# 5l1v3r1/gr-dvbt2ll

Hardware: NVIDIA B200
Metric: t2_baseband_msps (higher is better)
Workload: dtype u8/f32

## Files before the change

gr-dvbt2ll_b200/csrc/t2_capi.cu:

```cuda
#include "../../include/dvbt2ll_cuda.h"

#include <cuda_runtime.h>

#include <algorithm>
#include <cmath>
#include <cstdio>
#include <cstdlib>
#include <cstring>
#include <memory>
#include <mutex>
#include <string>
#include <vector>

#include "t2_kernels.cuh"
#include "t2_plan.h"

namespace {

thread_local std::string g_err;

int fail(int code, const std::string &msg) { g_err = msg; return code; }

#define CK(call)                                                                                  \
  do {                                                                                            \
// ... 280 lines not shown
struct BbHandle : dvbt2ll_handle {
  t2::BbPlan plan;
  DevBuf d_scr, d_crc, d_tab, d_cols, d_ib, d_ts, d_packed;
  int count, fec_block;
  uint8_t history[187];
  long long total_consumed;
  int *h_err;
  BbHandle() : dvbt2ll_handle(BB), count(0), fec_block(0), total_consumed(0), h_err(0) { std::memset(history, 0, sizeof(history)); }
  ~BbHandle() { if (h_err) cudaFreeHost(h_err); }
  void note_consumed(const uint8_t *in, long long used)
  {
    if (used >= 187) std::memcpy(history, in + used - 187, 187);
    else if (used > 0) {
      std::memmove(history, history + used, 187 - (size_t)used);
      std::memcpy(history + 187 - used, in, (size_t)used);
    }
  }

  int output_multiple() const { return plan.fec.nbch; }
  int in_item() const { return 1; }
  int out_item() const { return 1; }
  int forecast(int noutput) const
  {
    const int base = (noutput - 80 - (plan.fec.nbch - plan.fec.kbch)) / 8;
    return plan.mode == t2::INPUTMODE_NORMAL ? base : base + ((plan.fec.kbch - 80) / 8) / 187 + 1;
  }
  uint32_t crc_pos_mask[47][8];
  int dev_init()
  {
    std::vector<uint8_t> scr(plan.scramble);
    scr.resize((scr.size() + 7) & ~(size_t)3, 0);
    CK(upload(d_scr, scr));
    CK(upload(d_crc, std::vector<uint8_t>(plan.crc8_tab, plan.crc8_tab + 256)));
    std::vector<uint8_t> crc(1024);
    for (int x = 0; x < 256; x++) {
      uint8_t v = plan.crc8_tab[x];
      for (int k = 0; k < 4; k++) { crc[k * 256 + x] = v; v = plan.crc8_tab[v]; }
    }
    uint32_t crc_mask[8];
    for (int k = 0; k < 8; k++) {
      crc_mask[k] = 0;
      for (int i = 0; i < 4; i++)
        for (int j = 0; j < 8; j++)
          if ((crc[(3 - i) * 256 + (1 << j)] >> k) & 1) crc_mask[k] |= 1u << (8 * i + j);
    }
    {
      auto step = [&](uint32_t t) { uint32_t c = 0; for (int k = 0; k < 8; k++) c |= (uint32_t)(__builtin_popcount(t & crc_mask[k]) & 1) << k; return c; };
      std::memset(crc_pos_mask, 0, sizeof(crc_pos_mask));
      for (int j = 0; j < 47; j++)
        for (int bit = 0; bit < 32; bit++) {
          uint32_t v = step(1u << bit);
          for (int r = 0; r < 46 - j; r++) v = step(v);
          for (int k = 0; k < 8; k++) if ((v >> k) & 1u) crc_pos_mask[j][k] |= 1u << bit;
        }
      for (int k = 0; k < 8; k++) crc_pos_mask[0][k] &= 0xFFFFFF00u;
    }
    CK(upload(d_tab, plan.bch_byte_tab));
    CK(upload(d_cols, plan.bch_shift_cols));
    CK(upload(d_ib, plan.inband_bytes));
    if (!h_err) {
      CK(cudaHostAlloc((void **)&h_err, 16, cudaHostAllocMapped | cudaHostAllocPortable));
      std::memset(h_err, 0, 16);
    }
    return 0;
  }
  long long payload_bytes(int frames, int fb0) const
  {
    long long nb = 0;
    if (plan.inband) nb = (fb0 + frames + plan.fecblocks - 1) / plan.fecblocks - (fb0 + plan.fecblocks - 1) / plan.fecblocks;
    return (long long)frames * plan.payload_bytes - 13 * nb;
  }
  long long ts_needed(int frames) const
  {
    const long long P = payload_bytes(frames, fec_block);
    if (plan.mode == t2::INPUTMODE_NORMAL || P == 0) return P;
    const int t0 = (188 - count) % 188;
    const long long last = P - 1;
    return (last < t0 ? last : t0 + 1 + (last - t0) + (last - t0) / 187) + 1;
  }
  void fill_args(t2k::BbArgs &a, const uint8_t *d_ts_ptr, long long pitch, int channels, int frames, int count0,
                 int fb0, int hist_valid, uint8_t *d_out, int out_pitch)
  {
    a.ts = d_ts_ptr; a.ts_pitch = pitch; a.hist_valid = hist_valid; a.n_channels = channels; a.frames = frames;
    a.count0 = count0; a.fec_block0 = fb0;
    a.kbch = plan.fec.kbch; a.nbch = plan.fec.nbch; a.bch_r = plan.fec.bch_r; a.payload_bytes = plan.payload_bytes;
    a.mode = plan.mode; a.inband = plan.inband ? 1 : 0; a.fecblocks = plan.fecblocks;
    a.chunk_bytes = plan.chunk_bytes; a.lead_zero_bytes = plan.lead_zero_bytes;
    a.scramble = d_scr.as<uint8_t>(); a.crc8_tab = d_crc.as<uint8_t>(); a.bch_tab = d_tab.as<uint32_t>();
    std::memcpy(a.crc8_pos_mask, crc_pos_mask, sizeof(crc_pos_mask));
    a.bch_cols = d_cols.as<uint32_t>(); a.inband_bytes = d_ib.as<uint8_t>();
    a.out = d_out; a.out_pitch = out_pitch; a.sync_errors = h_err;
    a.ts_len = 0; a.out_len = (long long)channels * frames * out_pitch;
    a.out_group = 0; a.out_group_stride = 0; a.out_group_off = 0;
  }
  int work_device(const void *d_in, int ninput, void *d_out, int noutput, int *consumed, cudaStream_t s)
  {
    const int frames = noutput / plan.fec.nbch;
    if (consumed) *consumed = 0;
    if (frames < 1) return 0;
    const long long need = ts_needed(frames);
    if (ninput < need) return fail(DVBT2LL_ERR_SHORT, "bbheaderbch_bb: not enough input items");
    const int pitch = align16(plan.fec.nbch / 8);
    CK(d_packed.ensure((size_t)frames * pitch));
    t2k::BbArgs a;
    fill_args(a, (const uint8_t *)d_in, 0, 1, frames, count, fec_block, hist_on_device, d_packed.as<uint8_t>(), pitch);
    a.ts_len = ninput;
    t2k::launch_bb_bch(a, s);
    t2k::launch_unpack_bits(d_packed.as<uint8_t>(), pitch, plan.fec.nbch, (uint8_t *)d_out, frames, s);
    CK(cudaGetLastError());
    count = (int)((count + need) % 188);
    if (plan.inband) fec_block = (fec_block + frames) % plan.fecblocks;
    total_consumed += need;
    if (consumed) *consumed = (int)need;
    return frames * plan.fec.nbch;
  }
  int hist_on_device = 0;
  long long plan_get(const char *name, void *out, long long cap) const
  {
    std::string n(name);
    if (n == "bb.scramble") return copy_vec(plan.scramble, out, cap);
    if (n == "bb.crc8") return copy_out(plan.crc8_tab, 256, out, cap);
    if (n == "bb.bch_tab") return copy_vec(plan.bch_byte_tab, out, cap);
    if (n == "bb.bch_cols") return copy_vec(plan.bch_shift_cols, out, cap);
    if (n == "bb.inband") return copy_vec(plan.inband_bytes, out, cap);
    if (n == "bb.dims") {
      const int v[8] = { plan.fec.kbch, plan.fec.nbch, plan.fec.q, plan.fec.bch_r, plan.payload_bytes,
                         plan.chunk_bytes, plan.lead_zero_bytes, plan.fec.nldpc };
      return copy_out(v, sizeof(v), out, cap);
    }
    return -1;
  }
};

struct LdpcHandle : dvbt2ll_handle {
  t2::LdpcPlan plan;
  DevBuf d_rowptr, d_entries, d_in_packed, d_out_packed;
  int lane_per_row;
  LdpcHandle() : dvbt2ll_handle(LDPC), lane_per_row(0) {}
  int output_multiple() const { return plan.fec.nldpc; }
  int in_item() const { return 1; }
  int out_item() const { return 1; }
  int forecast(int noutput) const { return (noutput / plan.fec.nldpc) * plan.fec.nbch; }
  int dev_init()
  {
    CK(upload(d_rowptr, plan.row_ptr));
    CK(upload(d_entries, plan.entries));
    lane_per_row = ldpc_lane_per_row_default(plan.fec.nldpc, plan.fec.q);
    const char *e = std::getenv("DVBT2LL_LDPC_MODE");
    if (e && (e[0] == '0' || e[0] == '1')) lane_per_row = e[0] - '0';
    return 0;
  }
  static int ldpc_lane_per_row_default(int nldpc, int q)
  {
    return nldpc == 64800 ? (q >= 90 ? 1 : 0) : (q >= 18 ? 1 : 0);
  }
  void fill_args(t2k::LdpcArgs &a, const uint8_t *in, int in_pitch, uint8_t *out, int out_pitch, int frames)
  {
    a.in = in; a.in_pitch = in_pitch; a.out = out; a.out_pitch = out_pitch; a.frames = frames;
    a.nbch = plan.fec.nbch; a.nldpc = plan.fec.nldpc; a.q = plan.fec.q; a.groups = plan.groups;
    a.row_ptr = d_rowptr.as<uint16_t>(); a.entries = d_entries.as<uint32_t>();
    a.lane_per_row = lane_per_row;
    a.in_len = (long long)frames * in_pitch + 64; a.out_len = (long long)frames * out_pitch;
  }
  int work_device(const void *d_in, int ninput, void *d_out, int noutput, int *consumed, cudaStream_t s)
  {
    const int frames = noutput / plan.fec.nldpc;
    if (consumed) *consumed = 0;
    if (frames < 1) return 0;
    if (ninput < frames * plan.fec.nbch) return fail(DVBT2LL_ERR_SHORT, "ldpc: not enough input items");
    const int ip = align16(plan.fec.nbch / 8), op = align16(plan.fec.nldpc / 8);
    CK(d_in_packed.ensure((size_t)frames * ip + 64));
    CK(d_out_packed.ensure((size_t)frames * op + 16));
    t2k::launch_pack_bits((const uint8_t *)d_in, plan.fec.nbch, d_in_packed.as<uint8_t>(), ip, frames, s);
    t2k::LdpcArgs a;
    fill_args(a, d_in_packed.as<uint8_t>(), ip, d_out_packed.as<uint8_t>(), op, frames);
    t2k::launch_ldpc(a, s);
    t2k::launch_unpack_ldpc(d_out_packed.as<uint8_t>(), op, plan.fec.nbch, plan.fec.nldpc, plan.fec.q, (uint8_t *)d_out, frames, s);
    CK(cudaGetLastError());
    if (consumed) *consumed = frames * plan.fec.nbch;
    return frames * plan.fec.nldpc;
  }
  long long plan_get(const char *name, void *out, long long cap) const
  {
    std::string n(name);
    if (n == "ldpc.row_ptr") return copy_vec(plan.row_ptr, out, cap);
    if (n == "ldpc.entries") return copy_vec(plan.entries, out, cap);
    return -1;
  }
};

struct MapHandle : dvbt2ll_handle {
  t2::MapPlan plan;
  DevBuf d_bitsrc, d_lut, d_packed, d_qlut;
  MapHandle() : dvbt2ll_handle(MAP) {}
  int output_multiple() const { return plan.cell_size; }
  int in_item() const { return 1; }
  int out_item() const { return 8; }
  int forecast(int noutput) const { return (noutput / plan.cell_size) * plan.fec.nldpc; }
  int dev_init()
  {
    CK(upload(d_bitsrc, plan.bit_src));
    CK(upload(d_lut, plan.lut));
    if (!plan.qpsk_lut.empty()) CK(upload(d_qlut, plan.qpsk_lut));
    return 0;
  }
  void fill_args(t2k::MapArgs &a, const uint8_t *in, int in_pitch, float2 *out, int frames)
  {
    a.in = in; a.in_pitch = in_pitch; a.out = out; a.frames = frames;
    a.nldpc = plan.fec.nldpc; a.mod = plan.mod; a.cell_size = plan.cell_size; a.cyclic_delay = plan.cyclic_delay;
    a.bit_src = d_bitsrc.as<uint16_t>(); a.lut = d_lut.as<float2>();
    a.qpsk_lut = plan.qpsk_lut.empty() ? 0 : d_qlut.as<uint2>(); a.qpsk_lin_cells = a.qpsk_lut ? plan.qpsk_lin_cells : 0;
    a.qpsk_par_q = a.qpsk_lut ? plan.qpsk_par_q : 0; a.qpsk_nbch = plan.qpsk_nbch;
    a.ci_inv = 0; a.ci_inv4 = 0; a.ci_inv4_stride = 0; a.fec_shift = 0; a.fecblocks = 1; a.out16 = 0; a.out16_frame_stride = 0;
    a.in_len = (long long)frames * in_pitch; a.out_len = 0;
    a.ncol = plan.ncol;
    a.im_from_re = plan.im_from_re; a.im_mask_i = plan.im_mask_i; a.im_mask_q = plan.im_mask_q; a.im_flip = plan.im_flip;
    std::memcpy(a.col_of_bit, plan.col_of_bit, 16);
    std::memcpy(a.twist_of_col, plan.twist_of_col, 16);
  }
  int work_device(const void *d_in, int ninput, void *d_out, int noutput, int *consumed, cudaStream_t s)
  {
    const int frames = noutput / plan.cell_size;
    if (consumed) *consumed = 0;
    if (frames < 1) return 0;
    if (ninput < frames * plan.fec.nldpc) return fail(DVBT2LL_ERR_SHORT, "interleavermod_bc: not enough input items");
    const int ip = align16(plan.fec.nldpc / 8);
    CK(d_packed.ensure((size_t)frames * ip + 16));
    t2k::launch_pack_ldpc((const uint8_t *)d_in, plan.fec.nbch, plan.fec.nldpc, plan.fec.q, d_packed.as<uint8_t>(), ip, frames, s);
    t2k::MapArgs a;
    fill_args(a, d_packed.as<uint8_t>(), ip, (float2 *)d_out, frames);
    t2k::launch_map(a, s);
    CK(cudaGetLastError());
    if (consumed) *consumed = frames * plan.fec.nldpc;
    return frames * plan.cell_size;
  }
  long long plan_get(const char *name, void *out, long long cap) const
  {
    std::string n(name);
    if (n == "map.bit_src") return copy_vec(plan.bit_src, out, cap);
    if (n == "map.lut") return copy_vec(plan.lut, out, cap);
    if (n == "map.qpsk") { const int v[3] = { plan.qpsk_lin_cells, plan.qpsk_par_q, plan.qpsk_nbch }; return copy_out(v, sizeof(v), out, cap); }
    if (n == "map.im_from_re") { const int v[4] = { plan.im_from_re, (int)plan.im_mask_i, (int)plan.im_mask_q, (int)plan.im_flip }; return copy_out(v, sizeof(v), out, cap); }
    return -1;
  }
};

struct FrameHandle : dvbt2ll_handle {
  t2::FramePlan plan;
  DevBuf d_code, d_pool;
  int t2_frame_num;
  FrameHandle() : dvbt2ll_handle(FRAME), t2_frame_num(0) {}
  int output_multiple() const { return plan.mapped_items; }
  int in_item() const { return 8; }
  int out_item() const { return 8; }
  int forecast(int noutput) const { return plan.stream_items * (noutput / plan.mapped_items); }
  int dev_init()
  {
    CK(upload(d_code, plan.code));
    CK(upload(d_pool, plan.pool.cells));
    return 0;
  }
  int work_device(const void *d_in, int ninput, void *d_out, int noutput, int *consumed, cudaStream_t s)
  {
    const int frames = noutput / plan.mapped_items;
    if (consumed) *consumed = 0;
    if (frames < 1) return 0;
    if ((long long)ninput < (long long)frames * plan.stream_items)
      return fail(DVBT2LL_ERR_SHORT, "framemapperfint_cc: not enough input items");
    t2k::GatherArgs a;
    a.in = (const float2 *)d_in; a.in_stride = plan.stream_items;
    a.out = (float2 *)d_out; a.out_stride = plan.mapped_items;
    a.code = d_code.as<int32_t>(); a.n = plan.mapped_items; a.pool = d_pool.as<float2>();
    a.l1post_base = plan.pool.l1post_base; a.l1post_cells = plan.pool.l1post_cells; a.l1post_variants = plan.pool.l1post_variants;
    a.frames = frames; a.frame_idx0 = t2_frame_num;
    t2k::launch_gather(a, s);
    CK(cudaGetLastError());
    t2_frame_num = (t2_frame_num + frames) % plan.prm.t2frames;
    if (consumed) *consumed = frames * plan.stream_items;
    return frames * plan.mapped_items;
  }
  long long plan_get(const char *name, void *out, long long cap) const
  {
    std::string n(name);
    if (n == "frame.code") return copy_vec(plan.code, out, cap);
    if (n == "frame.pool") return copy_vec(plan.pool.cells, out, cap);
    if (n == "frame.cell_perm") return copy_vec(plan.cell_perm, out, cap);
    if (n == "frame.fec_shift") return copy_vec(plan.fec_shift, out, cap);
    if (n == "frame.ci_dst") return copy_vec(plan.ci_dst, out, cap);
    if (n == "frame.ti_src") return copy_vec(plan.ti_src, out, cap);
    if (n == "frame.dims") return dims_get(plan.dims, out, cap);
    if (n == "frame.info") {
      const int v[12] = { plan.cell_size, plan.stream_items, plan.mapped_items, plan.eta_mod, plan.n_post, plan.n_punc,
                          plan.dummy_cells, plan.pool.l1post_base, plan.pool.l1post_cells, plan.pool.l1post_variants,
                          plan.pool_dummy, plan.pool_zero };
      return copy_out(v, sizeof(v), out, cap);
    }
    return -1;
  }
};

struct OfdmDevice {
  DevBuf d_code, d_pool, d_p1, d_sinc, d_tw, d_tw_split, d_sym_flags;
  int log2_m, split;
  long long pool_stride;
  int init(const std::vector<int32_t> &code, const t2::CellPool &pool, const t2::OfdmPlan &op, bool c16 = false,
           const std::vector<uint8_t> *plp = 0, const int *tab_base = 0)
  {
    {
      const int nv = pool.l1post_variants > 0 ? pool.l1post_variants : 1;
      pool_stride = (long long)pool.cells.size();
      std::vector<t2::cfloat> rep((size_t)nv * pool.cells.size());
      for (int v = 0; v < nv; v++) {
        std::copy(pool.cells.begin(), pool.cells.end(), rep.begin() + (size_t)v * pool.cells.size());
        for (int i = 0; i < pool.l1post_cells; i++)
          rep[(size_t)v * pool.cells.size() + pool.l1post_base + i] = pool.cells[pool.l1post_base + (size_t)v * pool.l1post_cells + i];
      }
      CK(upload(d_pool, rep));
    }
    CK(upload(d_p1, op.p1));
    const int N = op.dims.fft_n;
    split = N > 16384 ? 2 : 1;
    const int M = N / split;
    log2_m = 0;
    while ((1 << log2_m) < M) log2_m++;
    const int L = op.dims.num_symbols, cps = op.dims.c_ps;
    std::vector<int> pos(M);
    for (int m = 0; m < M; m++) pos[m] = t2k::ofdm_table_index(t2k::ofdm_position_of_bin(m, log2_m), log2_m);
    std::vector<int32_t> code_pos((size_t)L * N, -1);
    std::vector<int32_t> sym_flags(L, 0);
// ... 96 lines not shown
  std::vector<uint16_t> c4((size_t)4 * *stride, 0);
  for (int k = 0; k < 4; k++)
    for (int j = 0; j + k < nc; j++) {
      const int c = ci_inv[j + k];
      c4[(size_t)k * *stride + j] = (uint16_t)(c + 2 * (c >> 6));
    }
  return c4;
}

struct ChainHandle : dvbt2ll_handle {
  BbHandle bb;
  LdpcHandle ldpc;
  MapHandle map;
  struct Set { BbHandle bb; LdpcHandle ldpc; MapHandle map; };
  std::unique_ptr<Set> xset[t2::MAX_PLP];
  DevBuf d_ci_inv_p[t2::MAX_PLP], d_ci_inv4_p[t2::MAX_PLP];
  int ci4_stride_p[t2::MAX_PLP];
  size_t bch_off[t2::MAX_PLP + 1], fec_off[t2::MAX_PLP + 1];
  std::vector<t2::cfloat> luts;
  int lut_tables, lut_base[t2::MAX_PLP], lut_single;
  int lut_copies;
  DevBuf d_luts;
  t2::FramePlan fplan;
  t2::OfdmPlan oplan;
  t2::Chain16Tables tables;
  OfdmDevice odev;
  DevBuf d_bch, d_fec, d_cells, d_ts_stage, d_out_stage, d_ci_inv, d_ci_inv4, d_fec_shift, d_run_desc, d_run_ptr, d_run_cnt, d_stage_bytes;
  int stage_cap, ci4_stride;
  int max_frames, device;
  int sink_fmt;
  float sink_gain;
  cudaStream_t stream2;
  int tr_iter;
  float tr_vclip, tr_tone_max;
  bool tr_built, tr_uploaded;
  t2::PaprTrPlan tr;
  DevBuf d_tr_set, d_tr_bins, d_tr_kernel, d_tr_tw, d_tr_stats, d_tr_scratch;
  int tr_frames;
  int last_frames;
  long long next_frame;
  bool timing;
  enum { TIMING_SLOTS = 64 };
  cudaEvent_t ev[TIMING_SLOTS][5];
  long long n_timed;
  ChainHandle() : dvbt2ll_handle(CHAIN), lut_tables(1), lut_single(0), lut_copies(0), max_frames(0), device(0), sink_fmt(0), sink_gain(1.0f), stream2(0), tr_iter(0), tr_vclip(0.f), tr_tone_max(0.f), tr_built(false), tr_uploaded(false), tr_frames(0), last_frames(0), next_frame(0), timing(false)
  {
    n_timed = 0;
    for (int s = 0; s < TIMING_SLOTS; s++) for (int i = 0; i < 5; i++) ev[s][i] = 0;
  }
  ~ChainHandle()
  {
    for (int s = 0; s < TIMING_SLOTS; s++) for (int i = 0; i < 5; i++) if (ev[s][i]) cudaEventDestroy(ev[s][i]);
    if (stream2) cudaStreamDestroy(stream2);
  }
  int enter() override
  {
    if (device >= 0) CK(cudaSetDevice(device));
    return ensure_device();
  }
  bool mixed() const { return fplan.plp_sets > 1; }
  BbHandle &bb_of(int plp) { const int s = fplan.plp_set[plp]; return s ? xset[s]->bb : bb; }
  const BbHandle &bb_of(int plp) const { const int s = fplan.plp_set[plp]; return s ? xset[s]->bb : bb; }
  LdpcHandle &ldpc_of(int plp) { const int s = fplan.plp_set[plp]; return s ? xset[s]->ldpc : ldpc; }
  MapHandle &map_of(int plp) { const int s = fplan.plp_set[plp]; return s ? xset[s]->map : map; }
  int bch_pitch(int plp) const { return align16(bb_of(plp).plan.fec.nbch / 8); }
  int fec_pitch(int plp) const { return align16(bb_of(plp).plan.fec.nldpc / 8); }
  int F() const { return fplan.prm.fecblocks; }
  int P() const { return fplan.num_plp; }
  int Fp(int plp) const { return fplan.plp_first_block[plp + 1] - fplan.plp_first_block[plp]; }
  long long cells16_stride() const { return ((long long)fplan.plp_chain_off[P()] + 7) & ~7LL; }
  long long stream_pos(long long frame, int plp = 0) const
  {
    const int fpl = Fp(plp);
    const long long j0 = frame * fpl;
    long long nb0 = 0;
    if (bb.plan.inband) nb0 = (j0 + fpl - 1) / fpl;
    const long long P = j0 * bb_of(plp).plan.payload_bytes - 13 * nb0;
    if (bb.plan.mode == t2::INPUTMODE_NORMAL || P == 0) return P;
    const long long last = P - 1;
    return 1 + last + last / 187 + 1;
  }
  long long ts_bytes(long long first_frame, int n_frames, int plp = 0) const { return stream_pos(first_frame + n_frames, plp) - stream_pos(first_frame, plp); }
  long long ts_bytes_max(long long first_frame, int n_frames) const
  {
    long long m = 0;
    for (int pl = 0; pl < P(); pl++) m = std::max(m, ts_bytes(first_frame, n_frames, pl));
    return m;
  }
  long long ts_per_frame() const { return ts_bytes(0, 1); }
  int output_multiple() const { return oplan.samples_per_frame; }
  int in_item() const { return 1; }
  int out_item() const { return sink_fmt ? 4 : 8; }
  int forecast(int noutput) const { return (int)(ts_per_frame() * (noutput / oplan.samples_per_frame)); }
  int dev_init()
  {
    bb.stream = 0; ldpc.stream = 0; map.stream = 0;
    int r;
    if ((r = bb.dev_init())) return r;
    if ((r = ldpc.dev_init())) return r;
    if ((r = map.dev_init())) return r;
    for (int s = 1; s < fplan.plp_sets; s++) {
      Set &x = *xset[s];
      x.bb.stream = 0; x.ldpc.stream = 0; x.map.stream = 0;
      if ((r = x.bb.dev_init()) || (r = x.ldpc.dev_init()) || (r = x.map.dev_init())) return r;
    }
    if ((r = odev.init(tables.code, tables.pool, oplan, true, &tables.plp, lut_tables > 1 ? lut_base : 0))) return r;
    CK(upload(d_ci_inv, fplan.cell_perm_inv));
    CK(upload(d_ci_inv4, make_ci_inv4(fplan.cell_perm_inv, &ci4_stride)));
    if (mixed()) {
      for (int pl = 0; pl < P(); pl++) {
        CK(upload(d_ci_inv_p[pl], fplan.plp_cell_perm_inv[pl]));
        CK(upload(d_ci_inv4_p[pl], make_ci_inv4(fplan.plp_cell_perm_inv[pl], &ci4_stride_p[pl])));
      }
      CK(upload(d_luts, luts));
    }
    CK(upload(d_fec_shift, fplan.fec_shift));
    CK(upload(d_run_desc, tables.run_desc));
    CK(upload(d_run_ptr, tables.run_ptr));
    CK(upload(d_run_cnt, tables.run_cnt));
    CK(upload(d_stage_bytes, tables.stage_bytes));
    stage_cap = (tables.max_slots + 7) & ~7;
    if ((size_t)(1 << odev.log2_m) * 8 * 17 / 16 + (size_t)stage_cap * 2 + 2048 + 96 + (size_t)(tables.max_runs + 2) * 8 > 227 * 1024)
      return fail(DVBT2LL_ERR_INVALID, "chain: the cells of one OFDM symbol do not fit the shared-memory staging area");
    const size_t nfec = (size_t)max_frames * F();
    bch_off[0] = fec_off[0] = 0;
    for (int pl = 0; pl < P(); pl++) {
      bch_off[pl + 1] = bch_off[pl] + (size_t)max_frames * Fp(pl) * bch_pitch(pl);
      fec_off[pl + 1] = fec_off[pl] + (size_t)max_frames * Fp(pl) * fec_pitch(pl);
    }
    if (mixed()) {
      CK(d_bch.ensure(bch_off[P()] + 64));
      CK(d_fec.ensure(fec_off[P()] + 64));
    }
    else CK(d_bch.ensure(nfec * align16(bb.plan.fec.nbch / 8) + 64));
    CK(d_cells.ensure((size_t)max_frames * cells16_stride() * sizeof(uint16_t) + 64));
    CK(cudaMemset(d_cells.p, 0, (size_t)max_frames * cells16_stride() * sizeof(uint16_t) + 64));
    for (int s = 0; s < TIMING_SLOTS; s++) for (int i = 0; i < 5; i++) CK(cudaEventCreate(&ev[s][i]));
    return 0;
  }
  int run(const void *d_ts, long long ts_pitch, int n_channels, int n_frames, long long first_frame, void *d_out, cudaStream_t s,
          int buf_frame = 0, int hist_valid = -1, int tr_frame0 = 0)
  {
    const int frames = n_channels * n_frames;
    if (frames < 1) return 0;
    if (buf_frame + frames > max_frames) return fail(DVBT2LL_ERR_INVALID, "chain: batch larger than max_frames given at create");
    const int nfec = frames * F();
    const int bp = align16(bb.plan.fec.nbch / 8), fp = align16(bb.plan.fec.nldpc / 8);
    cudaEvent_t *tev = ev[n_timed % TIMING_SLOTS];
    if (timing) cudaEventRecord(tev[0], s);
    uint8_t *bch_buf = d_bch.as<uint8_t>() + (size_t)buf_frame * F() * bp;
    if (!mixed()) CK(d_fec.ensure((size_t)max_frames * F() * fp + 64));
    uint8_t *fec_buf = d_fec.as<uint8_t>() + (size_t)buf_frame * F() * fp;
    uint16_t *cell_buf = d_cells.as<uint16_t>() + (size_t)buf_frame * cells16_stride();
    if (mixed()) run_plps(d_ts, ts_pitch, n_channels, n_frames, first_frame, cell_buf, s, buf_frame, hist_valid, tev);
    else {
    for (int pl = 0; pl < P(); pl++) {
      const int fpl = Fp(pl);
      const long long j0 = first_frame * fpl;
      const int fb0 = bb.plan.inband ? (int)(j0 % fpl) : 0;
      const int count0 = (int)(stream_pos(first_frame, pl) % 188);
      t2k::BbArgs ba;
      bb.fill_args(ba, (const uint8_t *)d_ts + (long long)pl * ts_pitch, ts_pitch * P(), n_channels, n_frames * fpl, count0, fb0,
                   hist_valid >= 0 ? hist_valid : (first_frame > 0 ? 1 : 0), bch_buf, bp);
      ba.fecblocks = fpl;
      ba.ts_len = ts_bytes(first_frame, n_frames, pl);
      ba.out_len = (long long)frames * F() * bp;
      if (P() > 1) { ba.out_group = fpl; ba.out_group_stride = F(); ba.out_group_off = fplan.plp_first_block[pl]; }
      t2k::launch_bb_bch(ba, s);
    }
    if (timing) cudaEventRecord(tev[1], s);
    t2k::LdpcArgs la;
    ldpc.fill_args(la, bch_buf, bp, fec_buf, fp, nfec);
    t2k::MapArgs ma;
    map.fill_args(ma, fec_buf, fp, 0, nfec);
    ma.out16 = cell_buf; ma.out16_frame_stride = cells16_stride();
    ma.ci_inv = d_ci_inv.as<uint16_t>(); ma.fec_shift = d_fec_shift.as<int32_t>(); ma.fecblocks = F();
    ma.ci_inv4 = d_ci_inv4.as<uint16_t>(); ma.ci_inv4_stride = ci4_stride;
    ma.out_len = (long long)frames * cells16_stride();
    t2k::launch_ldpc(la, s);
    if (timing) cudaEventRecord(tev[2], s);
    t2k::launch_map(ma, s);
    if (timing) cudaEventRecord(tev[3], s);
    }
    const bool tr_on = tr_iter > 0, tr_inplace = tr_on && sink_fmt == 0 && sink_gain == 1.0f;
    const long long spf = oplan.samples_per_frame;
    void *ofdm_out = d_out;
    if (tr_on) {
      int r = tr_upload();
      if (r) return r;
      CK(d_tr_stats.ensure((size_t)(tr_frame0 + frames) * oplan.dims.num_symbols * sizeof(int16_t)));
      if (!tr_inplace) {
        CK(d_tr_scratch.ensure((size_t)max_frames * spf * sizeof(float2)));
        ofdm_out = d_tr_scratch.as<float2>() + (size_t)buf_frame * spf;
      }
    }
    t2k::OfdmArgs oa;
    odev.fill(oa, oplan, tables.pool);
    oa.cells = 0; oa.cells_stride = cells16_stride();
    oa.cells16 = cell_buf; oa.run_desc = d_run_desc.as<int2>(); oa.run_ptr = d_run_ptr.as<int32_t>();
    oa.run_cnt = d_run_cnt.as<int32_t>(); oa.desc_cap = (tables.max_runs + 2) & ~1;
    oa.stage_bytes = d_stage_bytes.as<int32_t>(); oa.stage_cap = stage_cap; oa.lut_single = map.plan.im_from_re;
    oa.lut = map.d_lut.as<float2>(); oa.lut_n = 1 << map.plan.mod;
    if (mixed()) { oa.lut_single = lut_single; oa.lut = d_luts.as<float2>(); oa.lut_n = (int)luts.size(); oa.lut_tables = lut_tables; }
    oa.out = ofdm_out; oa.out_stride = oplan.samples_per_frame;
    oa.cells_len = (long long)frames * cells16_stride(); oa.out_len = (long long)frames * oplan.samples_per_frame;
    oa.out_fmt = sink_fmt; oa.sink_gain = sink_gain; oa.norm = oplan.normalization * sink_gain;
    if (ofdm_out != d_out) { oa.out_fmt = 0; oa.sink_gain = 1.0f; oa.norm = oplan.normalization; }
    oa.frames = frames; oa.frames_per_channel = n_frames;
    oa.frame_idx0 = (int)(first_frame % (tables.pool.l1post_variants > 0 ? tables.pool.l1post_variants : 1));
    lut_copies = t2k::launch_ofdm(oa, s);
    if (tr_on) {
      t2k::PaprArgs pa;
      pa.in = (const float2 *)ofdm_out; pa.out = d_out;
      pa.out_fmt = sink_fmt; pa.gain = sink_gain; pa.inplace = tr_inplace ? 1 : 0;
      pa.spf = spf; pa.fft_n = oplan.dims.fft_n; pa.gi = oplan.dims.gi; pa.num_symbols = oplan.dims.num_symbols; pa.frames = frames;
      pa.iterations = tr_iter; pa.vclip = tr_vclip; pa.tone_max = tr_tone_max;
      pa.tone_scale = (float)(1.0 / ((double)oplan.normalization * tr.tones));
      pa.tones = tr.tones; pa.sets = tr.sets;
      pa.sym_set = d_tr_set.as<int32_t>(); pa.bins = d_tr_bins.as<int32_t>();
      pa.kernel = d_tr_kernel.as<float2>(); pa.tone_tw = d_tr_tw.as<float2>();
      pa.stats = d_tr_stats.as<int16_t>() + (size_t)tr_frame0 * oplan.dims.num_symbols;
      pa.in_len = pa.out_len = (long long)frames * spf;
      t2k::launch_papr_tr(pa, s);
      tr_frames = tr_frame0 + frames;
    }
    if (timing) { cudaEventRecord(tev[4], s); n_timed++; }
    CK(cudaGetLastError());
    if (buf_frame == 0) last_frames = frames;
    return frames;
  }
  int tr_upload()
  {
    if (tr_uploaded) return 0;
    CK(upload(d_tr_set, tr.sym_set));
    CK(upload(d_tr_bins, tr.bins));
    CK(upload(d_tr_kernel, tr.kernel));
    CK(upload(d_tr_tw, tr.tone_tw));
    tr_uploaded = true;
    return 0;
  }
  void run_plps(const void *d_ts, long long ts_pitch, int n_channels, int n_frames, long long first_frame, uint16_t *cell_buf,
                cudaStream_t s, int buf_frame, int hist_valid, cudaEvent_t *tev)
  {
    const int frames = n_channels * n_frames;
    auto bch_buf = [&](int pl) { return d_bch.as<uint8_t>() + bch_off[pl] + (size_t)buf_frame * Fp(pl) * bch_pitch(pl); };
    auto fec_buf = [&](int pl) { return d_fec.as<uint8_t>() + fec_off[pl] + (size_t)buf_frame * Fp(pl) * fec_pitch(pl); };
    for (int pl = 0; pl < P(); pl++) {
      const int fpl = Fp(pl);
      const long long j0 = first_frame * fpl;
      t2k::BbArgs ba;
      bb_of(pl).fill_args(ba, (const uint8_t *)d_ts + (long long)pl * ts_pitch, ts_pitch * P(), n_channels, n_frames * fpl,
                          (int)(stream_pos(first_frame, pl) % 188), bb.plan.inband ? (int)(j0 % fpl) : 0,
                          hist_valid >= 0 ? hist_valid : (first_frame > 0 ? 1 : 0), bch_buf(pl), bch_pitch(pl));
      ba.fecblocks = fpl;
      ba.ts_len = ts_bytes(first_frame, n_frames, pl);
      t2k::launch_bb_bch(ba, s);
    }
    if (timing) cudaEventRecord(tev[1], s);
    for (int pl = 0; pl < P(); pl++) {
      t2k::LdpcArgs la;
      ldpc_of(pl).fill_args(la, bch_buf(pl), bch_pitch(pl), fec_buf(pl), fec_pitch(pl), frames * Fp(pl));
      t2k::launch_ldpc(la, s);
    }
    if (timing) cudaEventRecord(tev[2], s);
    for (int pl = 0; pl < P(); pl++) {
      t2k::MapArgs ma;
      map_of(pl).fill_args(ma, fec_buf(pl), fec_pitch(pl), 0, frames * Fp(pl));
      ma.out16 = cell_buf + fplan.plp_chain_off[pl]; ma.out16_frame_stride = cells16_stride();
      ma.ci_inv = d_ci_inv_p[pl].as<uint16_t>(); ma.fec_shift = d_fec_shift.as<int32_t>() + fplan.plp_first_block[pl];
      ma.fecblocks = Fp(pl);
      ma.ci_inv4 = d_ci_inv4_p[pl].as<uint16_t>(); ma.ci_inv4_stride = ci4_stride_p[pl];
      ma.im_from_re = lut_single;
      ma.out_len = (long long)frames * cells16_stride() - fplan.plp_chain_off[pl];
      t2k::launch_map(ma, s);
    }
    if (timing) cudaEventRecord(tev[3], s);
  }
  int work_device(const void *d_in, int ninput, void *d_out, int noutput, int *consumed, cudaStream_t s)
  {
    const int frames = noutput / oplan.samples_per_frame;
    if (consumed) *consumed = 0;
    if (frames < 1) return 0;
    const long long need = ts_bytes(next_frame, frames);
    if ((long long)ninput < need) return fail(DVBT2LL_ERR_SHORT, "chain: not enough input items");
    int r = run(d_in, 0, 1, frames, next_frame, d_out, s);
    if (r < 0) return r;
    next_frame += frames;
    if (consumed) *consumed = (int)need;
    return frames * oplan.samples_per_frame;
  }
  long long plan_get(const char *name, void *out, long long cap) const
  {
    std::string n(name);
    if (n == "chain.code") return copy_vec(tables.code, out, cap);
    if (n == "chain.pool") return copy_vec(tables.pool.cells, out, cap);
    if (n == "chain.run_desc") return copy_vec(tables.run_desc, out, cap);
    if (n == "chain.run_ptr") return copy_vec(tables.run_ptr, out, cap);
    if (n == "chain.run_cnt") return copy_vec(tables.run_cnt, out, cap);
    if (n == "chain.stage_bytes") return copy_vec(tables.stage_bytes, out, cap);
    if (n == "ofdm.sym_data_start") return copy_vec(oplan.sym_data_start, out, cap);
    if (n == "frame.framed") return copy_vec(fplan.framed, out, cap);
    if (n == "frame.pool") return copy_vec(fplan.pool.cells, out, cap);
    if (n == "frame.info") {
      const int v[12] = { fplan.cell_size, fplan.stream_items, fplan.mapped_items, fplan.eta_mod, fplan.n_post, fplan.n_punc,
                          fplan.dummy_cells, fplan.pool.l1post_base, fplan.pool.l1post_cells, fplan.pool.l1post_variants,
                          fplan.pool_dummy, fplan.pool_zero };
      return copy_out(v, sizeof(v), out, cap);
    }
    if (n == "frame.plp") {
      int v[2 + t2::MAX_PLP + 1] = { fplan.num_plp, fplan.l1post_sig_bits };
      for (int i = 0; i <= fplan.num_plp; i++) v[2 + i] = fplan.plp_first_block[i];
      return copy_out(v, sizeof(int) * (3 + fplan.num_plp), out, cap);
    }
    if (n == "frame.fi_src") return copy_vec(fplan.fi_src, out, cap);
    if (tr_built && n == "ofdm.tr_set") return copy_vec(tr.sym_set, out, cap);
    if (tr_built && n == "ofdm.tr_bins") return copy_vec(tr.bins, out, cap);
    if (tr_built && n == "ofdm.tr_kernel") return copy_vec(tr.kernel, out, cap);
    if (n == "frame.fec_shift") return copy_vec(fplan.fec_shift, out, cap);
    if (n == "frame.plp_cells") {
      int v[3 * t2::MAX_PLP];
      for (int i = 0; i < P(); i++) { v[3 * i] = fplan.plp_cell_size[i]; v[3 * i + 1] = fplan.plp_first_cell[i]; v[3 * i + 2] = fplan.plp_chain_off[i]; }
      return copy_out(v, sizeof(int) * 3 * P(), out, cap);
    }
    if (n == "chain.luts") {
      int v[3 + t2::MAX_PLP] = { lut_tables, mixed() ? lut_single : map.plan.im_from_re, lut_copies };
      for (int i = 0; i < P(); i++) v[3 + i] = mixed() ? lut_base[i] : 0;
      return copy_out(v, sizeof(int) * (3 + P()), out, cap);
    }
    long long r;
    if ((r = bb.plan_get(name, out, cap)) >= 0) return r;
    if ((r = ldpc.plan_get(name, out, cap)) >= 0) return r;
    if ((r = map.plan_get(name, out, cap)) >= 0) return r;
    if (n == "frame.code") return copy_vec(fplan.code, out, cap);
    if (n == "frame.ci_dst") return copy_vec(fplan.ci_dst, out, cap);
    if (n == "ofdm.code") return copy_vec(oplan.code, out, cap);
    if (n == "ofdm.dims") return dims_get(oplan.dims, out, cap);
    return -1;
  }
};

}

extern "C" {

const char *dvbt2ll_last_error(void) { return g_err.c_str(); }
#ifdef DVBT2LL_DEBUG_BOUNDS
const char *dvbt2ll_version(void) { return "dvbt2ll-b200 0.2 (sm_100a, bounds-checking debug build)"; }
#else
const char *dvbt2ll_version(void) { return "dvbt2ll-b200 0.2 (sm_100a)"; }
#endif
long long dvbt2ll_kernel_launches(void) { return t2k::kernel_launch_count(); }

int dvbt2ll_device_available(void)
{
  int n = 0;
  if (cudaGetDeviceCount(&n) != cudaSuccess) { cudaGetLastError(); return 0; }
  return n > 0;
}

int dvbt2ll_output_multiple(const dvbt2ll_handle *h) { return h ? h->output_multiple() : DVBT2LL_ERR_INVALID; }
int dvbt2ll_forecast(const dvbt2ll_handle *h, int noutput) { return h ? h->forecast(noutput) : DVBT2LL_ERR_INVALID; }
int dvbt2ll_warnings(const dvbt2ll_handle *h) { return h ? h->warnings : 0; }
void dvbt2ll_destroy(dvbt2ll_handle *h) { delete h; }

long long dvbt2ll_plan_get(const dvbt2ll_handle *h, const char *name, void *out, long long cap)
{
  if (!h || !name) return -1;
  return h->plan_get(name, out, cap);
}

int dvbt2ll_work_device(dvbt2ll_handle *h, const void *d_in, int ninput, void *d_out, int noutput, int *consumed, void *stream)
{
  if (!h) return fail(DVBT2LL_ERR_INVALID, "null handle");
  int r = h->enter();
  if (r) return r;
  if (h->kind == dvbt2ll_handle::BB) {
    BbHandle *b = static_cast<BbHandle *>(h);
    b->hist_on_device = b->total_consumed > 0 ? 1 : 0;
  }
  cudaStream_t s = stream ? (cudaStream_t)stream : h->stream;
  r = h->work_device(d_in, ninput, d_out, noutput, consumed, s);
  if (r >= 0 && !stream) CK(cudaStreamSynchronize(s));
  return r;
}

int dvbt2ll_work(dvbt2ll_handle *h, const void *in, int ninput, void *out, int noutput, int *consumed)
{
  if (!h) return fail(DVBT2LL_ERR_INVALID, "null handle");
  if (consumed) *consumed = 0;
  int r = h->enter();
  if (r) return r;
  const int om = h->output_multiple();
  const int frames = noutput / om;
  if (frames < 1) return 0;
  const int nout = frames * om;
  BbHandle *b = h->kind == dvbt2ll_handle::BB ? static_cast<BbHandle *>(h) : 0;
  ChainHandle *ch = h->kind == dvbt2ll_handle::CHAIN ? static_cast<ChainHandle *>(h) : 0;
  if (ch && ch->P() > 1) return fail(DVBT2LL_ERR_INVALID, "chain: a multi-PLP chain takes one TS per PLP: use dvbt2ll_chain_run_host / _run_device");
  if (ch) b = &ch->bb;
  long long need;
  if (ch) need = ch->ts_bytes(ch->next_frame, frames);
  else if (b) need = b->ts_needed(frames);
  else need = (long long)h->forecast(nout);
  if (ninput < need) return fail(DVBT2LL_ERR_SHORT, "not enough input items for the requested output");
  if (ch && frames > ch->max_frames) return fail(DVBT2LL_ERR_INVALID, "chain: more frames requested than max_frames given at create");
  DevBuf &d_in = h->stage_in;
  const size_t in_bytes = (size_t)need * h->in_item(), out_bytes = (size_t)nout * h->out_item();
  const size_t prefix = 192;
  std::shared_ptr<LinkRec> found_in = h->link_in;
  std::unique_lock<std::mutex> lk_in, lk_out;
  const bool auto_link = !ch && AutoLinks::get().enabled();
  if (auto_link && !h->link_out) {
    h->link_out = std::make_shared<LinkRec>();
    h->link_out->item = h->out_item();
    AutoLinks::get().add(h->link_out);
  }
  if (!found_in && auto_link && !b) {
    const uint8_t *ip = (const uint8_t *)in;
    std::vector<std::shared_ptr<LinkRec> > cand;
    if (std::shared_ptr<LinkRec> last = h->auto_in.lock()) cand.push_back(last);
    const size_t tried_first = cand.size();
    for (int pass = 0; pass < 2 && !found_in; pass++) {
      if (pass == 1) AutoLinks::get().snapshot(cand);
      for (size_t i = pass ? tried_first : 0; i < cand.size() && !found_in; i++) {
        LinkRec &L = *cand[i];
        if (cand[i] == h->link_out || L.item != h->in_item()) continue;
        std::unique_lock<std::mutex> g(L.m);
        for (int k = 0; k < LinkRec::NSLOT; k++) {
          const LinkRec::Slot &S = L.slot[k];
// ... 71 lines not shown
    b->hist_on_device = 1;
  }
  if (!resident) CK(h->copy_host(din, in, in_bytes, cudaMemcpyHostToDevice, s));
  int used = 0;
  if (ch) {
    r = ch->run(din, 0, 1, frames, ch->next_frame, d_out.p, s, 0, 1);
    if (r >= 0) { r = nout; used = (int)need; ch->next_frame += frames; }
  }
  else r = h->work_device(din, (int)need, d_out.p, nout, &used, s);
  if (r < 0) return r;
  if (resident) {
    if (!taken->taken_ev) CK(cudaEventCreateWithFlags(&taken->taken_ev, cudaEventDisableTiming));
    CK(cudaEventRecord(taken->taken_ev, s));
    taken->taken_valid = true;
    lk_in.unlock();
  }
  const bool lazy_out = h->link_out && h->link_out->lazy;
  if (!lazy_out) CK(h->copy_host(out, d_out.p, out_bytes, cudaMemcpyDeviceToHost, s));
  CK(cudaStreamSynchronize(s));
  if (b) {
    h->warnings = *b->h_err;
    b->note_consumed((const uint8_t *)in, used);
  }
  if (mine) {
    lk_out.lock();
    LinkRec &L = *h->link_out;
    mine->host = (const uint8_t *)out; mine->bytes = out_bytes; mine->valid = true;
    mine->pending = lazy_out; mine->taken_to = 0;
    L.next = (L.next + 1) % LinkRec::NSLOT;
  }
  if (consumed) *consumed = used;
  return r;
}

long long dvbt2ll_ts_sync(const unsigned char *ts, size_t n)
{
  if (!ts) return -1;
  for (size_t off = 0; off < 188 && off < n; off++) {
    int ok = 0;
    size_t q = off;
    for (; q < n && ok < 5; q += 188, ok++)
      if (ts[q] != 0x47) break;
    if (ok == 5 || (ok > 0 && q >= n)) return (long long)off;
  }
  return -1;
}
long long dvbt2ll_ts_fill(unsigned char *dst, size_t dst_bytes, const unsigned char *src, size_t src_bytes, long long pos)
{
  if (!dst) return -1;
  const long long whole = (long long)(src_bytes / 188) * 188;
  long long nulls = 0;
  for (size_t i = 0; i < dst_bytes; i++) {
    const long long q = pos + (long long)i;
    if (q < 0) dst[i] = 0;
    else if (q < whole && src) dst[i] = src[q];
    else {
      const int k = (int)(q % 188);
      dst[i] = k == 0 ? 0x47 : k == 1 ? 0x1F : k == 2 ? 0xFF : k == 3 ? 0x10 : 0xFF;
      nulls++;
    }
  }
  return nulls;
}

int dvbt2ll_copy_to_host(void *dst, const void *d_src, size_t bytes)
{
  CK(cudaMemcpy(dst, d_src, bytes, cudaMemcpyDeviceToHost));
  return 0;
}
int dvbt2ll_copy_to_device(void *d_dst, const void *src, size_t bytes)
{
  CK(cudaMemcpy(d_dst, src, bytes, cudaMemcpyHostToDevice));
  return 0;
}
void *dvbt2ll_device_alloc(size_t bytes)
{
  void *p = 0;
  if (cudaMalloc(&p, bytes) != cudaSuccess) { fail(DVBT2LL_ERR_CUDA, std::string("cudaMalloc: ") + cudaGetErrorString(cudaGetLastError())); return 0; }
  return p;
}
void dvbt2ll_device_free(void *p) { if (p) cudaFree(p); }
int dvbt2ll_device_count(void)
{
  int n = 0;
  if (cudaGetDeviceCount(&n) != cudaSuccess) { cudaGetLastError(); return 0; }
  return n;
}
int dvbt2ll_set_device(int device) { CK(cudaSetDevice(device)); return 0; }
void *dvbt2ll_stream_create(void)
{
  cudaStream_t s = 0;
  if (cudaStreamCreateWithFlags(&s, cudaStreamNonBlocking) != cudaSuccess) { fail(DVBT2LL_ERR_CUDA, "cudaStreamCreate failed"); cudaGetLastError(); return 0; }
  return (void *)s;
}
void dvbt2ll_stream_destroy(void *stream) { if (stream) cudaStreamDestroy((cudaStream_t)stream); }
int dvbt2ll_stream_synchronize(void *stream) { CK(cudaStreamSynchronize((cudaStream_t)stream)); return 0; }
int dvbt2ll_device_synchronize(void) { CK(cudaDeviceSynchronize()); return 0; }

void dvbt2ll_set_overfull_policy(int policy) { t2::set_overfull_policy(policy); }

void dvbt2ll_set_host_register(dvbt2ll_handle *h, int on) { if (h) h->pin_enabled = on != 0; }

int dvbt2ll_link(dvbt2ll_handle *producer, dvbt2ll_handle *consumer)
{
  if (!producer || !consumer || producer == consumer) return fail(DVBT2LL_ERR_INVALID, "link: two distinct handles needed");
  if (producer->out_item() != consumer->in_item()) return fail(DVBT2LL_ERR_INVALID, "link: item sizes differ");
  if (consumer->kind == dvbt2ll_handle::BB || consumer->kind == dvbt2ll_handle::CHAIN)
    return fail(DVBT2LL_ERR_INVALID, "link: a TS-consuming block keeps stream history in front of its input and cannot be a consumer");
  std::shared_ptr<LinkRec> L = std::make_shared<LinkRec>();
  L->item = producer->out_item();
  producer->link_out = L;
  consumer->link_in = L;
  return 0;
}

long long dvbt2ll_link_hits(const dvbt2ll_handle *consumer)
{
  if (!consumer) return 0;
  return consumer->link_in ? consumer->link_in->hits : consumer->auto_hits;
}

void dvbt2ll_set_auto_link(int on)
{
  AutoLinks &a = AutoLinks::get();
  std::lock_guard<std::mutex> g(a.m);
  a.on = on ? 1 : 0;
}

int dvbt2ll_link_lazy_host(dvbt2ll_handle *producer, int on)
{
  if (!producer || !producer->link_out) return fail(DVBT2LL_ERR_INVALID, "link_lazy_host: the handle is not the producer of a link");
  std::lock_guard<std::mutex> g(producer->link_out->m);
  producer->link_out->lazy = on != 0;
  return 0;
}

long long dvbt2ll_link_late_writes(const dvbt2ll_handle *producer) { return (producer && producer->link_out) ? producer->link_out->late_writes : 0; }

dvbt2ll_handle *dvbt2ll_bbheaderbch_create(int framesize, int rate, int mode, int inband, int fecblocks, int tsrate)
{
  BbHandle *h = new BbHandle();
  std::string err;
  if (mode != t2::INPUTMODE_NORMAL && mode != t2::INPUTMODE_HIEFF) { delete h; fail(DVBT2LL_ERR_INVALID, "bbheaderbch_bb: unknown input mode"); return 0; }
  if (!t2::build_bb_plan(framesize, rate, mode, inband, fecblocks, tsrate, &h->plan, &err)) { delete h; fail(DVBT2LL_ERR_INVALID, err); return 0; }
  return h;
}

dvbt2ll_handle *dvbt2ll_ldpc_create(int framesize, int rate)
{
  LdpcHandle *h = new LdpcHandle();
  std::string err;
  if (!t2::build_ldpc_plan(framesize, rate, &h->plan, &err)) { delete h; fail(DVBT2LL_ERR_INVALID, err); return 0; }
  return h;
}

dvbt2ll_handle *dvbt2ll_interleavermod_create(int framesize, int rate, int constellation, int rotation)
{
  MapHandle *h = new MapHandle();
  std::string err;
  if (!t2::build_map_plan(framesize, rate, constellation, rotation, &h->plan, &err)) { delete h; fail(DVBT2LL_ERR_INVALID, err); return 0; }
  return h;
}

dvbt2ll_handle *dvbt2ll_framemapperfint_create(int framesize, int rate, int constellation, int rotation, int fecblocks,
                                               int tiblocks, int carriermode, int fftsize, int guardinterval,
                                               int l1constellation, int pilotpattern, int t2frames, int numdatasyms,
                                               int paprmode, int version, int preamble, int inputmode,
                                               int reservedbiasbits, int l1scrambled, int inband)
{
  FrameHandle *h = new FrameHandle();
  std::string err;
  t2::FrameParams p = { framesize, rate, constellation, rotation, fecblocks, tiblocks, carriermode, fftsize, guardinterval,
                        l1constellation, pilotpattern, t2frames, numdatasyms, paprmode, version, preamble, inputmode,
                        reservedbiasbits, l1scrambled, inband };
  if (!t2::build_frame_plan(p, &h->plan, &err)) { delete h; fail(DVBT2LL_ERR_INVALID, err); return 0; }
  if (h->plan.overfull) { h->warnings = 1; g_err = "Frame Mapper, too many FEC blocks in T2 frame."; }
  return h;
}

dvbt2ll_handle *dvbt2ll_pilotgenp1insert_create(int carriermode, int fftsize, int pilotpattern, int guardinterval,
                                                int numdatasyms, int paprmode, int version, int preamble,
                                                int misogroup, int equalization, int bandwidth, int vlength)
{
  OfdmHandle *h = new OfdmHandle();
  std::string err;
  t2::OfdmParams p = { carriermode, fftsize, pilotpattern, guardinterval, numdatasyms, paprmode, version, preamble,
                       misogroup, equalization, bandwidth, vlength };
  if (!t2::build_ofdm_plan(p, &h->plan, &err)) { delete h; fail(DVBT2LL_ERR_INVALID, err); return 0; }
  return h;
}

static dvbt2ll_handle *chain_create(const dvbt2ll_chain_params *c, int num_plp, const int *plp_fecblocks, int max_frames, int device)
{
  if (!c || max_frames < 1) { fail(DVBT2LL_ERR_INVALID, "chain: bad arguments"); return 0; }
  if (num_plp < 1 || num_plp > t2::MAX_PLP || (num_plp > 1 && !plp_fecblocks)) { fail(DVBT2LL_ERR_INVALID, "chain: number of PLPs out of range"); return 0; }
  ChainHandle *h = new ChainHandle();
  std::string err;
  h->max_frames = max_frames; h->device = device;
  int fecblocks = c->fecblocks;
  if (num_plp > 1) {
    fecblocks = 0;
    for (int p = 0; p < num_plp; p++) fecblocks += plp_fecblocks[p];
  }
  t2::FrameParams fp = { c->framesize, c->rate, c->constellation, c->rotation, fecblocks, c->tiblocks, c->carriermode,
                         c->fftsize, c->guardinterval, c->l1constellation, c->pilotpattern, c->t2frames, c->numdatasyms,
                         c->paprmode, c->version, c->preamble, c->inputmode, c->reservedbiasbits, c->l1scrambled, c->inband };
  fp.num_plp = num_plp;
  for (int p = 0; p < num_plp && num_plp > 1; p++) fp.plp_fecblocks[p] = plp_fecblocks[p];
  t2::OfdmParams op = { c->carriermode, c->fftsize, c->pilotpattern, c->guardinterval, c->numdatasyms, c->paprmode,
                        c->version, c->preamble, c->misogroup, c->equalization, c->bandwidth, c->vlength };
  bool ok = true;
  ok = ok && t2::build_bb_plan(c->framesize, c->rate, c->inputmode, c->inband, fecblocks, c->tsrate, &h->bb.plan, &err);
  ok = ok && t2::build_ldpc_plan(c->framesize, c->rate, &h->ldpc.plan, &err);
  ok = ok && t2::build_map_plan(c->framesize, c->rate, c->constellation, c->rotation, &h->map.plan, &err);
  ok = ok && t2::build_frame_plan(fp, &h->fplan, &err);
  ok = ok && t2::build_ofdm_plan(op, &h->oplan, &err);
  ok = ok && t2::compose_chain16(h->fplan, h->oplan, &h->tables, &err);
  if (!ok) { delete h; fail(DVBT2LL_ERR_INVALID, err); return 0; }
  if (h->fplan.overfull) { h->warnings = 1; g_err = "Frame Mapper, too many FEC blocks in T2 frame."; }
  return h;
}

dvbt2ll_handle *dvbt2ll_chain_create_plps(const dvbt2ll_chain_params *c, int num_plp, const dvbt2ll_plp_params *plp, int max_frames,
                                          int device)
{
  if (!c || !plp || max_frames < 1) { fail(DVBT2LL_ERR_INVALID, "chain: bad arguments"); return 0; }
  if (num_plp < 1 || num_plp > t2::MAX_PLP) { fail(DVBT2LL_ERR_INVALID, "chain: number of PLPs out of range"); return 0; }
  int fecblocks = 0;
  for (int p = 0; p < num_plp; p++) {
    if (plp[p].fecblocks < 1 || plp[p].fecblocks > 1023) { fail(DVBT2LL_ERR_INVALID, "chain: FEC blocks of a PLP out of range"); return 0; }
    fecblocks += plp[p].fecblocks;
  }
  std::unique_ptr<ChainHandle> h(new ChainHandle());
  std::string err;
  h->max_frames = max_frames; h->device = device;
  t2::FrameParams fp = { plp[0].framesize, plp[0].rate, plp[0].constellation, plp[0].rotation, fecblocks, c->tiblocks,
                         c->carriermode, c->fftsize, c->guardinterval, c->l1constellation, c->pilotpattern, c->t2frames,
                         c->numdatasyms, c->paprmode, c->version, c->preamble, c->inputmode, c->reservedbiasbits,
                         c->l1scrambled, c->inband };
  fp.num_plp = num_plp;
  fp.plp_modcod = 1;
  for (int p = 0; p < num_plp; p++) {
    fp.plp_fecblocks[p] = plp[p].fecblocks;
    fp.plp_framesize[p] = plp[p].framesize; fp.plp_rate[p] = plp[p].rate;
    fp.plp_constellation[p] = plp[p].constellation; fp.plp_rotation[p] = plp[p].rotation;
  }
  t2::OfdmParams op = { c->carriermode, c->fftsize, c->pilotpattern, c->guardinterval, c->numdatasyms, c->paprmode,
                        c->version, c->preamble, c->misogroup, c->equalization, c->bandwidth, c->vlength };
  bool ok = t2::build_frame_plan(fp, &h->fplan, &err);
  for (int s = 0; ok && s < h->fplan.plp_sets; s++) {
    int p = 0;
    while (h->fplan.plp_set[p] != s) p++;
    if (s) h->xset[s].reset(new ChainHandle::Set());
    BbHandle &bb = s ? h->xset[s]->bb : h->bb;
    LdpcHandle &ldpc = s ? h->xset[s]->ldpc : h->ldpc;
    MapHandle &map = s ? h->xset[s]->map : h->map;
    ok = ok && t2::build_bb_plan(plp[p].framesize, plp[p].rate, c->inputmode, c->inband, fecblocks, c->tsrate, &bb.plan, &err);
    ok = ok && t2::build_ldpc_plan(plp[p].framesize, plp[p].rate, &ldpc.plan, &err);
    ok = ok && t2::build_map_plan(plp[p].framesize, plp[p].rate, plp[p].constellation, plp[p].rotation, &map.plan, &err);
  }
  ok = ok && t2::build_ofdm_plan(op, &h->oplan, &err);
  ok = ok && t2::compose_chain16(h->fplan, h->oplan, &h->tables, &err);
  if (!ok) { fail(DVBT2LL_ERR_INVALID, err); return 0; }
  if (h->mixed()) {
    std::vector<int> order;
    for (int p = 0; p < num_plp; p++) order.push_back(p);
    std::stable_sort(order.begin(), order.end(), [&](int x, int y) { return plp[x].constellation > plp[y].constellation; });
    h->lut_tables = 0;
    h->lut_single = 1;
    for (size_t i = 0; i < order.size(); i++) {
      const int p = order[i];
      const t2::MapPlan &mp = h->map_of(p).plan;
      h->lut_single &= mp.im_from_re;
      size_t j = 0;
      while (j < i && !(plp[order[j]].constellation == plp[p].constellation && plp[order[j]].rotation == plp[p].rotation)) j++;
      if (j < i) { h->lut_base[p] = h->lut_base[order[j]]; continue; }
      h->lut_base[p] = (int)h->luts.size();
      h->luts.insert(h->luts.end(), mp.lut.begin(), mp.lut.end());
      h->lut_tables++;
    }
    h->luts.resize((h->luts.size() + 15) & ~(size_t)15);
    if (h->luts.size() - 1 > t2k::OFDM_CODE_TAB_MAX) { fail(DVBT2LL_ERR_INVALID, "chain: constellation tables too large"); return 0; }
  }
  return h.release();
}

dvbt2ll_handle *dvbt2ll_chain_create(const dvbt2ll_chain_params *c, int max_frames, int device)
{
  return chain_create(c, 1, 0, max_frames, device);
}

dvbt2ll_handle *dvbt2ll_chain_create_multiplp(const dvbt2ll_chain_params *c, int num_plp, const int *plp_fecblocks, int max_frames, int device)
{
  return chain_create(c, num_plp, plp_fecblocks, max_frames, device);
}

static ChainHandle *as_chain(const dvbt2ll_handle *h)
{
  return (h && h->kind == dvbt2ll_handle::CHAIN) ? static_cast<ChainHandle *>(const_cast<dvbt2ll_handle *>(h)) : 0;
}

long long dvbt2ll_chain_ts_bytes_per_frame(const dvbt2ll_handle *h) { ChainHandle *c = as_chain(h); return c ? c->ts_per_frame() : -1; }
long long dvbt2ll_chain_ts_bytes(const dvbt2ll_handle *h, long long first_frame, int n_frames)
{
  ChainHandle *c = as_chain(h);
  return c ? c->ts_bytes(first_frame, n_frames) : -1;
// ... 175 lines not shown
```

gr-dvbt2ll_b200/csrc/t2_kernels.cu:

```cuda
#include "t2_kernels.cuh"

#include <atomic>

#ifdef DVBT2LL_DEBUG_BOUNDS
#include <cstdio>
#define BND(ok)                                                                                                   \
  do {                                                                                                            \
    if (!(ok)) {                                                                                                  \
      printf("DVBT2LL bounds violation: %s (t2_kernels.cu:%d, block %d thread %d)\n", #ok, __LINE__, (int)blockIdx.x, (int)threadIdx.x); \
      __trap();                                                                                                   \
    }                                                                                                             \
  } while (0)
#else
#define BND(ok) do { } while (0)
#endif

namespace t2k {

static std::atomic<long long> g_launches(0);
long long kernel_launch_count() { return g_launches.load(); }
static inline void count_launch() { g_launches.fetch_add(1); }
void count_extra_launch() { count_launch(); }

constexpr int MAX_DEVICES = 64;
static inline int current_device()
{
  int dev = 0;
  cudaGetDevice(&dev);
  return (dev < 0 || dev >= MAX_DEVICES) ? 0 : dev;
}

static inline int sm_count()
{
  static int n[MAX_DEVICES];
  const int dev = current_device();
  if (!n[dev]) {
    int v = 0;
    cudaDeviceGetAttribute(&v, cudaDevAttrMultiProcessorCount, dev);
    n[dev] = v > 0 ? v : 148;
  }
  return n[dev];
}

template <class K>
static inline void allow_smem(K k, int bytes, bool (&done)[MAX_DEVICES])
{
  const int dev = current_device();
  if (done[dev]) return;
  cudaFuncSetAttribute(k, cudaFuncAttributeMaxDynamicSharedMemorySize, bytes);
  done[dev] = true;
}

__device__ __forceinline__ uint32_t bswap32(uint32_t x) { return __byte_perm(x, 0, 0x0123); }
__device__ __forceinline__ uint32_t window32(const uint32_t *w, int p)
{
  const int k = p >> 5;
  return __funnelshift_l(w[k + 1], w[k], p & 31);
}

constexpr int BB_MAX_WARPS = 32;

__device__ __forceinline__ int multiples_in(int a, int b, int m)
{
  return (b + m - 1) / m - (a + m - 1) / m;
}

__device__ __forceinline__ long long hem_ts_index(long long P, int c0)
{
  const int t0 = (188 - c0) % 188;
  if (P < t0) return P;
  const long long pp = P - t0;
  return t0 + 1 + pp + pp / 187;
}

template <bool W6>
__global__ void __launch_bounds__(BB_MAX_WARPS * 32) k_bb_bch(const BbArgs a)
{
  extern __shared__ __align__(16) uint8_t smem_raw[];
  constexpr int NW = W6 ? 6 : 5;
  uint32_t *s_ntab = reinterpret_cast<uint32_t *>(smem_raw);
  uint32_t *s_cols = s_ntab + 4 * 16 * NW * 32;
  uint8_t *s_crc8 = reinterpret_cast<uint8_t *>(s_cols + 6 * 32 * 6);
  uint8_t *s_buf = s_crc8 + 256;
  const int nbytes = a.nbch / 8, msg_bytes = a.kbch / 8;
  constexpr int HIST = 192;
  const int buf_pitch = ((nbytes + 15) & ~15) + HIST;

#pragma unroll 1
  for (int i0 = threadIdx.x; i0 < 4 * 16 * NW * 32; i0 += 8 * blockDim.x) {
    uint32_t v[8];
#pragma unroll
    for (int u = 0; u < 8; u++) {
      const int i = i0 + u * blockDim.x;
      const int w = (i >> 5) % NW, kn = (i >> 5) / NW, k = kn >> 4, n = kn & 15;
      v[u] = i < 4 * 16 * NW * 32 ? __ldg(a.bch_tab + ((k >> 1) * 256 + (n << (4 * (k & 1)))) * 6 + w) : 0u;
    }
#pragma unroll
    for (int u = 0; u < 8; u++) {
      const int i = i0 + u * blockDim.x;
      if (i < 4 * 16 * NW * 32) s_ntab[i] = v[u];
    }
  }
#pragma unroll 4
  for (int i = threadIdx.x; i < 6 * 32 * 6; i += blockDim.x) s_cols[i] = __ldg(a.bch_cols + i);
  for (int i = threadIdx.x; i < 256; i += blockDim.x) s_crc8[i] = a.crc8_tab[i];
  __syncthreads();
  const uint8_t *S1 = s_crc8;

  const int warp = threadIdx.x >> 5, lane = threadIdx.x & 31;
  uint8_t *buf = s_buf + warp * buf_pitch + HIST;
  uint32_t *bufw = reinterpret_cast<uint32_t *>(buf);
  const int total = a.n_channels * a.frames;
  const int D = a.payload_bytes;
  const bool hem = a.mode != 0;
  const uint32_t *scr32 = reinterpret_cast<const uint32_t *>(a.scramble);

  const int nwarps = blockDim.x >> 5;
  for (int job = blockIdx.x * nwarps + warp; job < total; job += gridDim.x * nwarps) {
    const int c = job / a.frames, j = job - c * a.frames;
    const uint8_t *ts = a.ts + (long long)c * a.ts_pitch;
    const int nb = a.inband ? multiples_in(a.fec_block0, a.fec_block0 + j, a.fecblocks) : 0;
    const bool ib = a.inband && ((a.fec_block0 + j) % a.fecblocks == 0);
    const long long P0 = (long long)j * D - 13LL * nb;
    const int Dj = D - (ib ? 13 : 0);
    long long t_start;
    if (!hem) t_start = P0;
    else t_start = P0 == 0 ? 0 : hem_ts_index(P0 - 1, a.count0) + 1;
    const int count = (int)((a.count0 + t_start) % 188);

    BND(10 + Dj + (ib ? 13 : 0) <= msg_bytes && msg_bytes + a.bch_r / 8 == nbytes && nbytes <= buf_pitch - HIST);
    BND(a.out_len == 0 || a.out_group != 0 || (long long)(job + 1) * a.out_pitch <= a.out_len + (a.out_pitch - nbytes));
    if (!hem) {
      const uint8_t *src = ts + P0;
      BND(a.ts_len == 0 || (P0 >= 0 && P0 + Dj <= a.ts_len));
      {
        const int nj = job + gridDim.x * nwarps;
        if (nj < total) {
          const int nc = nj / a.frames, njj = nj - nc * a.frames;
          const int nnb = a.inband ? multiples_in(a.fec_block0, a.fec_block0 + njj, a.fecblocks) : 0;
          const uint8_t *nsrc = a.ts + (long long)nc * a.ts_pitch + ((long long)njj * D - 13LL * nnb);
          for (int o = lane * 128; o < D; o += 32 * 128) asm volatile("prefetch.global.L2 [%0];" ::"l"(nsrc + o));
        }
      }
      if (lane < 2) buf[10 + lane] = src[lane];
      const int w_end = (10 + Dj) >> 2;
      {
        const uintptr_t ad = reinterpret_cast<uintptr_t>(src + 2);
        const uint32_t *wp = reinterpret_cast<const uint32_t *>(ad & ~(uintptr_t)3);
        const int sh = (int)(ad & 3) * 8;
        const int last = w_end - 4;
        if (last >= 0)
        for (int w0 = lane; w0 <= last; w0 += 128) {
          uint32_t lo[4], hi[4];
#pragma unroll
          for (int u = 0; u < 4; u++) {
            const int k = min(w0 + 32 * u, last);
            lo[u] = __ldg(wp + k);
            hi[u] = __ldg(wp + k + (sh ? 1 : 0));
          }
#pragma unroll
          for (int u = 0; u < 4; u++)
            if (w0 + 32 * u <= last) bufw[3 + w0 + 32 * u] = __funnelshift_r(lo[u], hi[u], sh);
        }
      }
      for (int i = 4 * w_end - 10 + lane; i < Dj; i += 32) buf[10 + i] = src[i];
      for (int k = 1 + lane; k <= 187; k += 32) buf[10 - k] = (P0 - k >= 0 || a.hist_valid) ? src[-k] : (uint8_t)0;
    }
    else {
      BND(a.ts_len == 0 || hem_ts_index(P0 + Dj - 1, a.count0) < a.ts_len);
      for (int i = lane; i < Dj; i += 32) buf[10 + i] = ts[hem_ts_index(P0 + i, a.count0)];
      const long long t_end = hem_ts_index(P0 + Dj - 1, a.count0);
      const int first = (int)((188 - (a.count0 + t_start) % 188) % 188);
      for (long long t = t_start + first + 188LL * lane; t <= t_end; t += 188LL * 32)
        if (ts[t] != 0x47) atomicAdd(a.sync_errors, 1);
    }
    __syncwarp();
    uint8_t my_crc[2] = { 0, 0 };
    const int i0 = (188 - count) % 188;
    if (!hem) {
#pragma unroll
      for (int rnd = 0; rnd < 2; rnd++) {
        const int si = i0 + 188 * (lane + 32 * rnd);
        if (si < Dj) {
          if (buf[10 + si] != 0x47) atomicAdd(a.sync_errors, 1);
          const uint8_t *p = buf + 10 + si - 188;
          BND(10 + si - 188 >= -HIST && si < Dj);
          const uint32_t *pw = reinterpret_cast<const uint32_t *>(reinterpret_cast<uintptr_t>(p) & ~(uintptr_t)3);
          const int sh = (int)(reinterpret_cast<uintptr_t>(p) & 3) * 8;
          uint32_t lo = pw[0];
          uint32_t acc[8] = { 0u, 0u, 0u, 0u, 0u, 0u, 0u, 0u };
#pragma unroll
          for (int st = 0; st < 47; st++) {
            const uint32_t hi = pw[st + 1];
            const uint32_t t = __funnelshift_r(lo, hi, sh);
            lo = hi;
#pragma unroll
            for (int k = 0; k < 8; k++) acc[k] ^= t & a.crc8_pos_mask[st][k];
          }
          uint32_t crc = 0;
#pragma unroll
          for (int k = 0; k < 8; k++) crc |= (__popc(acc[k]) & 1u) << k;
          my_crc[rnd] = (uint8_t)crc;
        }
      }
    }
    __syncwarp();
    if (!hem) {
#pragma unroll
      for (int rnd = 0; rnd < 2; rnd++) {
        const int si = i0 + 188 * (lane + 32 * rnd);
        if (si < Dj) buf[10 + si] = my_crc[rnd];
      }
    }
    if (lane == 0) {
      uint8_t h[10];
      h[0] = 0xF0;
      h[1] = 0x00;
      const int upl = hem ? 0 : 188 * 8, dfl = a.kbch - 80 - (ib ? 104 : 0);
      const int syncd = count ? (188 - count) * 8 : 0;
      h[2] = (uint8_t)(upl >> 8); h[3] = (uint8_t)upl;
      h[4] = (uint8_t)(dfl >> 8); h[5] = (uint8_t)dfl;
      h[6] = hem ? 0x00 : 0x47;
      h[7] = (uint8_t)(syncd >> 8); h[8] = (uint8_t)syncd;
      uint8_t crc = 0;
      for (int i = 0; i < 9; i++) crc = S1[crc ^ h[i]];
      h[9] = hem ? (crc ^ 1) : crc;
      for (int i = 0; i < 10; i++) buf[i] = h[i];
    }
    if (ib)
      for (int i = lane; i < 13; i += 32) buf[10 + Dj + i] = a.inband_bytes[i];
    __syncwarp();
    for (int w = lane; w < (msg_bytes + 3) >> 2; w += 32) bufw[w] ^= __ldg(scr32 + w);
    __syncwarp();

    uint32_t r0 = 0, r1 = 0, r2 = 0, r3 = 0, r4 = 0, r5 = 0;
    {
      int s = lane * a.chunk_bytes - a.lead_zero_bytes;
      const int e = s + a.chunk_bytes;
      if (s < 0) s = 0;
      int i = s;
      const uint32_t *nt = s_ntab + lane;
      constexpr int ROW = NW * 32;
      auto step8 = [&](uint32_t byte) {
        const uint32_t x = (r0 >> 24) ^ byte;
        const uint32_t *t1 = nt + (16 + (x >> 4)) * ROW, *t0 = nt + (x & 15u) * ROW;
        r0 = ((r0 << 8) | (r1 >> 24)) ^ t1[0] ^ t0[0];
        r1 = ((r1 << 8) | (r2 >> 24)) ^ t1[32] ^ t0[32];
        r2 = ((r2 << 8) | (r3 >> 24)) ^ t1[64] ^ t0[64];
        r3 = ((r3 << 8) | (r4 >> 24)) ^ t1[96] ^ t0[96];
        r4 = ((r4 << 8) | (W6 ? r5 >> 24 : 0u)) ^ t1[128] ^ t0[128];
        if (W6) r5 = (r5 << 8) ^ t1[NW * 32 - 32] ^ t0[NW * 32 - 32];
      };
      auto step16 = [&](uint32_t half) {
        const uint32_t x = (r0 >> 16) ^ half;
        const uint32_t *t3 = nt + (48 + (x >> 12)) * ROW, *t2 = nt + (32 + ((x >> 8) & 15u)) * ROW,
                       *t1 = nt + (16 + ((x >> 4) & 15u)) * ROW, *t0 = nt + (x & 15u) * ROW;
        r0 = ((r0 << 16) | (r1 >> 16)) ^ t3[0] ^ t2[0] ^ t1[0] ^ t0[0];
        r1 = ((r1 << 16) | (r2 >> 16)) ^ t3[32] ^ t2[32] ^ t1[32] ^ t0[32];
        r2 = ((r2 << 16) | (r3 >> 16)) ^ t3[64] ^ t2[64] ^ t1[64] ^ t0[64];
        r3 = ((r3 << 16) | (r4 >> 16)) ^ t3[96] ^ t2[96] ^ t1[96] ^ t0[96];
        r4 = ((r4 << 16) | (W6 ? r5 >> 16 : 0u)) ^ t3[128] ^ t2[128] ^ t1[128] ^ t0[128];
        if (W6) r5 = (r5 << 16) ^ t3[NW * 32 - 32] ^ t2[NW * 32 - 32] ^ t1[NW * 32 - 32] ^ t0[NW * 32 - 32];
      };
      for (; (i & 3) && i < e; i++) step8(buf[i]);
      for (; i + 4 <= e; i += 4) {
        const uint32_t mw = bufw[i >> 2];
        step16(__byte_perm(mw, 0u, 0x4401u));
        step16(__byte_perm(mw, 0u, 0x4423u));
      }
      for (; i < e; i++) step8(buf[i]);
    }
    uint32_t c0 = __shfl_sync(0xffffffffu, r0, 0), c1 = __shfl_sync(0xffffffffu, r1, 0),
             c2 = __shfl_sync(0xffffffffu, r2, 0), c3 = __shfl_sync(0xffffffffu, r3, 0),
             c4 = __shfl_sync(0xffffffffu, r4, 0), c5 = __shfl_sync(0xffffffffu, r5, 0);
    {
      constexpr int NW = W6 ? 6 : 5;
      uint32_t col[NW][NW];
#pragma unroll
      for (int w = 0; w < NW; w++)
#pragma unroll
        for (int k = 0; k < NW; k++) col[w][k] = s_cols[(w * 32 + lane) * 6 + k];
      for (int i = 1; i < 32; i++) {
        uint32_t n[6];
        n[5] = 0;
#pragma unroll
        for (int w = 0; w < NW; w++) {
          uint32_t x = (c0 & col[w][0]) ^ (c1 & col[w][1]) ^ (c2 & col[w][2]) ^ (c3 & col[w][3]) ^ (c4 & col[w][4]);
          if (W6) x ^= c5 & col[w][NW - 1];
          n[w] = __ballot_sync(0xffffffffu, __popc(x) & 1);
        }
        c0 = n[0] ^ __shfl_sync(0xffffffffu, r0, i);
        c1 = n[1] ^ __shfl_sync(0xffffffffu, r1, i);
        c2 = n[2] ^ __shfl_sync(0xffffffffu, r2, i);
        c3 = n[3] ^ __shfl_sync(0xffffffffu, r3, i);
        c4 = n[4] ^ __shfl_sync(0xffffffffu, r4, i);
        c5 = n[5] ^ __shfl_sync(0xffffffffu, r5, i);
      }
    }
    if (lane < a.bch_r / 8) {
      const int wsel = lane >> 2;
      const uint32_t word = wsel == 0 ? c0 : wsel == 1 ? c1 : wsel == 2 ? c2 : wsel == 3 ? c3 : wsel == 4 ? c4 : c5;
      buf[msg_bytes + lane] = (uint8_t)(word >> (24 - 8 * (lane & 3)));
    }
    __syncwarp();
    const long long oslot = a.out_group ? (long long)(job / a.out_group) * a.out_group_stride + a.out_group_off + job % a.out_group : job;
    uint8_t *o = a.out + oslot * a.out_pitch;
    const int nw = nbytes >> 2;
    uint32_t *ow = reinterpret_cast<uint32_t *>(o);
    for (int i = lane; i < nw; i += 32) ow[i] = bufw[i];
    for (int i = (nw << 2) + lane; i < nbytes; i += 32) o[i] = buf[i];
    __syncwarp();
  }
}

void launch_bb_bch(const BbArgs &a, cudaStream_t s)
{
  const int nbytes = a.nbch / 8;
  const int buf_pitch = ((nbytes + 15) & ~15) + 192;
  const bool w6 = a.bch_r > 160;
  const size_t fixed = (size_t)4 * 16 * (w6 ? 6 : 5) * 32 * 4 + 6 * 32 * 6 * 4 + 256;
  const int total = a.n_channels * a.frames;
  if (total < 1) return;
  static bool attr6[MAX_DEVICES], attr5[MAX_DEVICES];
  allow_smem(k_bb_bch<true>, 227 * 1024, attr6);
  allow_smem(k_bb_bch<false>, 227 * 1024, attr5);
  int warps = BB_MAX_WARPS;
  while (warps > 4 && fixed + (size_t)warps * buf_pitch > 227 * 1024) warps -= 4;
  const int spread = (total + sm_count() - 1) / sm_count();
  if (spread < warps) warps = spread < 1 ? 1 : spread;
  else {
    const int rounds = (spread + warps - 1) / warps;
    warps = (spread + rounds - 1) / rounds;
  }
  const size_t smem = fixed + (size_t)warps * buf_pitch;
  int blocks = (total + warps - 1) / warps;
  const int cap = sm_count();
  if (blocks > cap) blocks = cap;
  if (w6) k_bb_bch<true><<<blocks, warps * 32, smem, s>>>(a);
  else k_bb_bch<false><<<blocks, warps * 32, smem, s>>>(a);
  count_launch();
}

constexpr int LDPC_WARPS = 3;

__device__ __forceinline__ uint32_t window32_be(const uint32_t *w, int p)
{
  const int k = p >> 5;
  return __funnelshift_l(bswap32(w[k + 1]), bswap32(w[k]), p & 31);
}

__device__ __forceinline__ uint32_t be32_at(const uint32_t *w, int off)
{
  const int k = off >> 2;
  return __byte_perm(__ldg(w + k), __ldg(w + k + 1), 0x0123u + 0x1111u * (unsigned)(off & 3));
}

__global__ void __launch_bounds__(LDPC_WARPS * 32, 8) k_ldpc(const LdpcArgs a, int warp_words, int cw_words)
{
  extern __shared__ __align__(16) uint8_t smem_raw[];
  uint32_t *s_all = reinterpret_cast<uint32_t *>(smem_raw);
  const int warp = threadIdx.x >> 5, lane = threadIdx.x & 31;
  uint32_t *rows = s_all + warp * warp_words;
  uint32_t *ext = rows + cw_words;
  const int q = a.q, G = a.groups;
  const int info_bytes = a.nbch / 8;

  for (int job = blockIdx.x * LDPC_WARPS + warp; job < a.frames; job += gridDim.x * LDPC_WARPS) {
    const uint8_t *in = a.in + (long long)job * a.in_pitch;
    uint8_t *out = a.out + (long long)job * a.out_pitch;
    const uint32_t *cw = reinterpret_cast<const uint32_t *>(in);
    BND(a.in_len == 0 || (long long)job * a.in_pitch + 45 * G + 8 <= a.in_len);
    BND(a.out_len == 0 || (long long)job * a.out_pitch + a.nldpc / 8 <= a.out_len);
    BND(45 * G == info_bytes && warp_words >= G * 13 + q * 12);
    {
      uint32_t *ow = reinterpret_cast<uint32_t *>(out);
      const int nw = info_bytes >> 2;
      for (int i = lane; i < nw; i += 256) {
        uint32_t v[8];
#pragma unroll
        for (int u = 0; u < 8; u++) v[u] = __ldg(cw + min(i + 32 * u, nw - 1));
#pragma unroll
        for (int u = 0; u < 8; u++) if (i + 32 * u < nw) ow[i + 32 * u] = v[u];
      }
      for (int b = (nw << 2) + lane; b < info_bytes; b += 32) out[b] = __ldg(in + b);
    }
    for (int idx0 = lane; idx0 < G * 13; idx0 += 128) {
      uint32_t v[4], h[4];
      int wsel[4];
#pragma unroll
      for (int u = 0; u < 4; u++) {
        const int idx = min(idx0 + 32 * u, G * 13 - 1);
        const int g = idx / 13, w = idx - g * 13;
        wsel[u] = w;
        v[u] = be32_at(cw, 45 * g + (w == 12 ? 3 : 4 * w));
        h[u] = be32_at(cw, 45 * g);
      }
#pragma unroll
      for (int u = 0; u < 4; u++)
        if (idx0 + 32 * u < G * 13) ext[idx0 + 32 * u] = wsel[u] == 11 ? (v[u] & 0xFF000000u) | (h[u] >> 8) : v[u];
    }
    __syncwarp();
    if (a.lane_per_row) {
      for (int t = lane; t < q; t += 32) {
        uint32_t acc[12];
#pragma unroll
        for (int w = 0; w < 12; w++) acc[w] = 0u;
        const int e1 = a.row_ptr[t + 1];
        for (int e = a.row_ptr[t]; e < e1; e++) {
          const uint32_t en = __ldg(a.entries + e);
          BND((int)(en & 0xffffu) < G && (en >> 16) < 360u);
          const uint32_t *eg = ext + (en & 0xffffu) * 13;
          int p = (en >> 16) ? 360 - (int)(en >> 16) : 0;
#pragma unroll
          for (int w = 0; w < 12; w++) {
            acc[w] ^= window32(eg, p);
            p += 32;
            if (p >= 360) p -= 360;
          }
        }
        acc[11] &= 0xFF000000u;
#pragma unroll
        for (int w = 0; w < 12; w++) rows[t * 12 + w] = acc[w];
      }
    }
    else
    for (int idx = lane; idx < q * 12; idx += 32) {
      const int t = idx / 12, w = idx - t * 12;
      uint32_t acc = 0;
      const int e1 = a.row_ptr[t + 1];
      int e = a.row_ptr[t];
      for (; e + 4 <= e1; e += 4) {
        uint32_t en[4];
#pragma unroll
        for (int u = 0; u < 4; u++) en[u] = __ldg(a.entries + e + u);
#pragma unroll
        for (int u = 0; u < 4; u++) {
          int p = 32 * w - (int)(en[u] >> 16);
          if (p < 0) p += 360;
          BND((int)(en[u] & 0xffffu) < G && (en[u] >> 16) < 360u && p >= 0 && p < 360);
          acc ^= window32(ext + (en[u] & 0xffffu) * 13, p);
        }
      }
      for (; e < e1; e++) {
        const uint32_t en = __ldg(a.entries + e);
        int p = 32 * w - (int)(en >> 16);
        if (p < 0) p += 360;
        BND((int)(en & 0xffffu) < G && (en >> 16) < 360u && p >= 0 && p < 360);
        acc ^= window32(ext + (en & 0xffffu) * 13, p);
      }
      if (w == 11) acc &= 0xFF000000u;
      rows[idx] = acc;
    }
    __syncwarp();
    if (lane < 12) {
      uint32_t run = 0;
      for (int t = 0; t < q; t++) { run ^= rows[t * 12 + lane]; rows[t * 12 + lane] = run; }
    }
    __syncwarp();
    uint32_t E = 0;
    {
      uint32_t x = lane < 12 ? rows[(q - 1) * 12 + lane] : 0;
      x ^= x >> 1; x ^= x >> 2; x ^= x >> 4; x ^= x >> 8; x ^= x >> 16;
      uint32_t par = x & 1u, carry = par;
#pragma unroll
      for (int d = 1; d < 16; d <<= 1) {
        const uint32_t o = __shfl_up_sync(0xffffffffu, carry, d);
        if (lane >= d) carry ^= o;
      }
      carry ^= par;
      E = (x >> 1) ^ (carry ? 0xFFFFFFFFu : 0u);
      if (lane == 11) E &= 0xFF000000u;
    }
    for (int i0 = 0; i0 < q * 12; i0 += 32) {
      const int idx = i0 + lane;
      const uint32_t ew = __shfl_sync(0xffffffffu, E, idx % 12);
      if (idx < q * 12) rows[idx] ^= ew;
    }
    __syncwarp();
    if ((info_bytes & 3) == 0) {
      uint32_t *pw = reinterpret_cast<uint32_t *>(out + info_bytes);
      const int nwp = (q * 360) >> 5;
      for (int j = lane; j < nwp; j += 32) {
        const int P = j << 5;
        const int t = P / 360, o = P - t * 360;
        uint32_t v = window32(rows + t * 12, o);
        const int n1 = 360 - o;
        if (n1 < 32) v = (v & ~(0xFFFFFFFFu >> n1)) | (rows[(t + 1) * 12] >> n1);
        pw[j] = bswap32(v);
      }
      for (int b = (nwp << 2) + lane; b < q * 45; b += 32) {
        const int t = b / 45, bb = b - t * 45;
        out[info_bytes + b] = (uint8_t)(rows[t * 12 + (bb >> 2)] >> (24 - 8 * (bb & 3)));
      }
    }
    else {
      for (int b = lane; b < q * 45; b += 32) {
        const int t = b / 45, bb = b - t * 45;
        out[info_bytes + b] = (uint8_t)(rows[t * 12 + (bb >> 2)] >> (24 - 8 * (bb & 3)));
      }
    }
    __syncwarp();
  }
}

void launch_ldpc(const LdpcArgs &a, cudaStream_t s)
{
  const int cw_words = a.q * 12 + 4;
  const int warp_words = (a.groups * 13 + cw_words + 3) & ~3;
  const size_t smem = (size_t)LDPC_WARPS * warp_words * 4;
  if (a.frames < 1) return;
  static bool attr[MAX_DEVICES];
  allow_smem(k_ldpc, 200 * 1024, attr);
  int per_sm = 1;
  cudaOccupancyMaxActiveBlocksPerMultiprocessor(&per_sm, k_ldpc, LDPC_WARPS * 32, smem);
  if (per_sm < 1) per_sm = 1;
  const int blocks = (a.frames + LDPC_WARPS - 1) / LDPC_WARPS;
  k_ldpc<<<blocks, LDPC_WARPS * 32, smem, s>>>(a, warp_words, cw_words);
  count_launch();
}

constexpr int MAP_THREADS = 128;

template <int J>
__device__ __forceinline__ void transpose32_stage(uint32_t (&A)[32])
{
  constexpr uint32_t m = J == 16 ? 0x0000FFFFu : J == 8 ? 0x00FF00FFu : J == 4 ? 0x0F0F0F0Fu : J == 2 ? 0x33333333u : 0x55555555u;
#pragma unroll
  for (int k = 0; k < 32; k++) {
    if ((k & J) == 0) {
      const uint32_t t = (A[k] ^ (A[k + J] >> J)) & m;
      A[k] ^= t;
      A[k + J] ^= t << J;
    }
  }
}

__device__ __forceinline__ void transpose32(uint32_t (&A)[32])
{
  transpose32_stage<16>(A);
  transpose32_stage<8>(A);
  transpose32_stage<4>(A);
  transpose32_stage<2>(A);
  transpose32_stage<1>(A);
}

template <bool QTR, int NCOL = 0>
__device__ __forceinline__ void map_body(const MapArgs &a, const int f, const uint32_t *u, const float2 *lut, uint16_t *cw,
                                         const int shift)
{
  const int mod = a.mod, Nc = a.cell_size;
  const bool tilde = a.im_from_re != 0;
  const uint32_t tI = a.im_mask_i * 0x01010101u, tQ = a.im_mask_q * 0x01010101u, tF = a.im_flip * 0x01010101u;
  auto tilde4 = [&](uint32_t w) -> uint32_t { return tilde ? ((((w << 1) & tI) | ((w >> 1) & tQ)) ^ tF) : w; };
  auto tilde1 = [&](uint32_t w) -> uint32_t { return tilde4(w) & 0xFFu; };
  if constexpr (NCOL != 0) {
    const int rows = a.nldpc / NCOL;
    const int groups = (rows + 31) >> 5;
    for (int g = threadIdx.x; g < groups; g += blockDim.x) {
      const int d0 = g << 5;
      uint32_t A[32];
#pragma unroll
      for (int y = 0; y < 32; y++) A[y] = 0;
#pragma unroll
      for (int y = 16; y < 32; y++) {
        const int rho = y - (32 - NCOL);
        if (rho >= 0) {
          int s0 = d0 - a.twist_of_bit[rho];
          if (s0 < 0) s0 += rows;
          const int base = a.base_of_bit[rho];
          const int n1 = rows - s0;
          uint32_t w = window32_be(u, base + s0);
          if (n1 < 32) w = (w & ~(0xFFFFFFFFu >> n1)) | (window32_be(u, base) >> n1);
          A[y] = w;
        }
      }
      transpose32(A);
      const uint32_t mask = (1u << mod) - 1u;
      const int xs = a.cyclic_delay ? 8 : 0;
      uint32_t wprev = 0;
      if (NCOL == 2 * mod) {
        uint32_t *dst = reinterpret_cast<uint32_t *>(cw + 2 * d0 + 2 * g);
#pragma unroll
        for (int i = 0; i < 32; i += 2) {
          const uint32_t p0 = A[i], p1 = A[i + 1];
          const uint32_t w = (p0 >> mod) | ((p0 & mask) << 8) | ((p1 >> mod) << 16) | ((p1 & mask) << 24);
          const uint32_t wt = tilde4(w), X = __funnelshift_l(wprev, wt, xs);
          dst[i] = __byte_perm(w, X, 0x5140u);
          dst[i + 1] = __byte_perm(w, X, 0x7362u);
          wprev = wt;
        }
      }
      else {
        uint32_t *dst = reinterpret_cast<uint32_t *>(cw + d0 + 2 * (g >> 1));
#pragma unroll
        for (int i = 0; i < 32; i += 4) {
          const uint32_t w = (A[i] & mask) | ((A[i + 1] & mask) << 8) | ((A[i + 2] & mask) << 16) | ((A[i + 3] & mask) << 24);
          const uint32_t wt = tilde4(w), X = __funnelshift_l(wprev, wt, xs);
          dst[i >> 1] = __byte_perm(w, X, 0x5140u);
          dst[(i >> 1) + 1] = __byte_perm(w, X, 0x7362u);
          wprev = wt;
        }
      }
    }
    if (a.cyclic_delay) {
      __syncthreads();
      const int run = NCOL == 2 * mod ? 64 : 32;
      for (int c = threadIdx.x * run; c < Nc; c += blockDim.x * run) {
        const int pc = c == 0 ? Nc - 1 : c - 1;
        reinterpret_cast<uint8_t *>(cw)[2 * (c + 2 * (c >> 6)) + 1] = (uint8_t)tilde1(cw[pc + 2 * (pc >> 6)]);
      }
    }
  }
  else if (mod == 2 && (Nc & 3) == 0) {
    const uint8_t *ub = reinterpret_cast<const uint8_t *>(u);
    const int lin = a.qpsk_lin_cells;
    for (int wi = threadIdx.x; wi < (lin >> 4); wi += blockDim.x) {
      const uint32_t W = u[wi];
      uint32_t *dst = reinterpret_cast<uint32_t *>(cw + 16 * wi + 2 * (wi >> 2));
#pragma unroll
      for (int k = 0; k < 4; k++) {
        const uint2 cd = __ldg(a.qpsk_lut + ((W >> (8 * k)) & 255u));
        dst[2 * k] = cd.x;
        dst[2 * k + 1] = cd.y;
      }
    }
    const int gen_end = QTR && a.qpsk_par_q > 0 ? (a.qpsk_nbch >> 1) : Nc;
    for (int c = lin + 4 * threadIdx.x; c < gen_end; c += 4 * blockDim.x) {
      const uint4 pp = __ldg(reinterpret_cast<const uint4 *>(a.bit_src) + (c >> 2));
      const uint32_t w[4] = { pp.x, pp.y, pp.z, pp.w };
      uint32_t code[4];
#pragma unroll
      for (int k = 0; k < 4; k++) {
        const uint32_t p0 = w[k] & 0xFFFFu, p1 = w[k] >> 16;
        const uint32_t v = (((ub[p0 >> 3] >> (7 - (p0 & 7))) & 1u) << 1) | ((ub[p1 >> 3] >> (7 - (p1 & 7))) & 1u);
        code[k] = v | (tilde1(v) << 8);
      }
      uint32_t *dst = reinterpret_cast<uint32_t *>(cw + c + 2 * (c >> 6));
      dst[0] = code[0] | (code[1] << 16);
      dst[1] = code[2] | (code[3] << 16);
    }
    if (QTR && a.qpsk_par_q > 0) {
      const int q = a.qpsk_par_q, nbch = a.qpsk_nbch, par0 = nbch >> 1;
      const int tr = (q + 31) >> 5;
      const bool have = (int)threadIdx.x < tr * 12;
      const int t0 = ((int)threadIdx.x / 12) << 5, s0 = ((int)threadIdx.x % 12) << 5;
      uint32_t A[32];
      if (have) {
#pragma unroll
        for (int y = 0; y < 32; y++) A[y] = t0 + y < q ? window32_be(u, nbch + 360 * (t0 + y) + s0) : 0u;
        transpose32(A);
      }
      __syncthreads();
      uint32_t *nat = const_cast<uint32_t *>(u);
      const int nat_words = ((q * 360 + 31) >> 5) + 1;
      for (int i = threadIdx.x; i < nat_words; i += blockDim.x) nat[i] = 0u;
      __syncthreads();
      if (have) {
        const int nv = min(32, q - t0);
        const uint32_t vmask = nv >= 32 ? 0xFFFFFFFFu : ~(0xFFFFFFFFu >> nv);
#pragma unroll
        for (int i = 0; i < 32; i++) {
          if (s0 + i < 360) {
            const uint32_t word = A[i] & vmask;
            const int P = q * (s0 + i) + t0, sh = P & 31;
            atomicOr(nat + (P >> 5), word >> sh);
            if (sh) atomicOr(nat + (P >> 5) + 1, word << (32 - sh));
          }
        }
      }
      __syncthreads();
      const int npar = Nc - par0;
// ... 666 lines not shown
  for (int b = 0; b < G::GPB; b++) {
    const int g = g0 + b * T;
    if (R0 == 4) {
      const int4 q4 = __ldg(reinterpret_cast<const int4 *>(code) + g);
      c[b][0] = q4.x; c[b][1 % R0] = q4.y; c[b][2 % R0] = q4.z; c[b][3 % R0] = q4.w;
    }
    else if (R0 == 8) {
      const int4 q4 = __ldg(reinterpret_cast<const int4 *>(code) + 2 * g), q5 = __ldg(reinterpret_cast<const int4 *>(code) + 2 * g + 1);
      c[b][0] = q4.x; c[b][1 % R0] = q4.y; c[b][2 % R0] = q4.z; c[b][3 % R0] = q4.w;
      c[b][4 % R0] = q5.x; c[b][5 % R0] = q5.y; c[b][6 % R0] = q5.z; c[b][7 % R0] = q5.w;
    }
    else if (R0 == 16) {
#pragma unroll
      for (int q = 0; q < 4; q++) {
        const int4 q4 = __ldg(reinterpret_cast<const int4 *>(code) + q * G::GROUPS + g);
        c[b][(4 * q) % R0] = q4.x; c[b][(4 * q + 1) % R0] = q4.y; c[b][(4 * q + 2) % R0] = q4.z; c[b][(4 * q + 3) % R0] = q4.w;
      }
    }
    else if (R0 == 2) {
      const int2 q2 = __ldg(reinterpret_cast<const int2 *>(code) + g);
      c[b][0] = q2.x; c[b][1 % R0] = q2.y;
    }
    else c[b][0] = __ldg(code + g);
  }
}

struct FillSmem {
  uint32_t stage_s;
  uint32_t lut_lane_s;
  uint32_t im_ofs;
  uint32_t spool_m8_s;
  uint32_t esh;
};

template <int LOG2M, int T, bool C16, bool POOL, bool SINC, bool MT = false>
__device__ __forceinline__ void ofdm_fill(float2 *x, const int32_t *__restrict__ code, const float *__restrict__ sinc,
                                          int (&c)[FillGeom<LOG2M, T>::GPB][FillGeom<LOG2M, T>::R0], const float2 *__restrict__ cells,
                                          const float2 *__restrict__ pool, const FillSmem fs, int stage_cap_dbg = 0, int lut_n_dbg = 0)
{
  typedef FillGeom<LOG2M, T> G;
  constexpr int R0 = G::R0, GPB = G::GPB;
#pragma unroll 1
  for (int g0 = threadIdx.x; g0 < G::GROUPS; g0 += G::STEP) {
    float2 v[GPB][R0];
#pragma unroll
    for (int b = 0; b < GPB; b++)
#pragma unroll
      for (int r = 0; r < R0; r++) {
        const int cc = c[b][r];
        if (C16) {
          const unsigned off = POOL && cc < 0 ? 0u : (unsigned)cc & 0x1FFFFu;
          BND(cc < 0 || (MT ? (unsigned)cc - 0x20000u < OFDM_CODE_SMALL_POOL : cc >= 0x20000) || off + 2 <= 2u * (unsigned)stage_cap_dbg);
          unsigned sc;
          asm volatile("ld.shared.u16 %0, [%1];" : "=r"(sc) : "r"(fs.stage_s + off));
          float2 val;
          if constexpr (MT) {
            const unsigned tb = POOL && cc < 0 ? 0u : (unsigned)cc >> OFDM_CODE_TAB_SHIFT;
            BND(tb + (sc & 255u) < (unsigned)lut_n_dbg && tb + (sc >> 8) < (unsigned)lut_n_dbg);
            asm volatile("ld.shared.f32 %0, [%1];" : "=f"(val.x) : "r"(fs.lut_lane_s + ((tb + (sc & 255u)) << fs.esh)));
            asm volatile("ld.shared.f32 %0, [%1];" : "=f"(val.y) : "r"(fs.lut_lane_s + fs.im_ofs + ((tb + (sc >> 8)) << fs.esh)));
          }
          else {
            asm volatile("ld.shared.f32 %0, [%1];" : "=f"(val.x) : "r"(fs.lut_lane_s + ((sc & 255u) << fs.esh)));
            asm volatile("ld.shared.f32 %0, [%1];" : "=f"(val.y) : "r"(fs.lut_lane_s + fs.im_ofs + ((sc >> 8) << fs.esh)));
          }
          if (MT ? (unsigned)cc - 0x20000u < OFDM_CODE_SMALL_POOL : cc >= 0x20000) asm volatile("ld.shared.v2.f32 {%0, %1}, [%2];" : "=f"(val.x), "=f"(val.y) : "r"(fs.spool_m8_s + ((unsigned)cc >> 14)));
          if (POOL && cc < 0) val = __ldg(pool + (cc & 0x7FFFFFFF));
          v[b][r] = val;
        }
        else {
          const float2 *base = cc >= 0 ? cells : pool;
          v[b][r] = __ldg(base + (cc >= 0 ? cc : ~cc));
        }
      }
    if (g0 + G::STEP < G::GROUPS) fill_load_codes<LOG2M, T>(code, g0 + G::STEP, c);
#pragma unroll
    for (int b = 0; b < GPB; b++) {
      const int g = g0 + b * T;
      if (SINC) {
#pragma unroll
        for (int r = 0; r < R0; r++) {
          const float sf = __ldg(sinc + (R0 == 16 ? (((r >> 2) * G::GROUPS + g) * 4 + (r & 3)) : g * R0 + r));
          v[b][r] = __fmul2_rn(v[b][r], make_float2(sf, sf));
        }
      }
      if (R0 > 1) dft_reg<R0>(v[b]);
      float2 *xb = x + padx(g * R0);
#pragma unroll
      for (int k = 0; k < R0; k++) xb[k] = v[b][bitrev_c(k, R0)];
    }
  }
}

constexpr int OFDM_PARK_COLS = 256;

template <int NCOLS>
__device__ __forceinline__ void tmem_alloc(uint32_t dst_s)
{
  asm volatile("tcgen05.alloc.cta_group::1.sync.aligned.shared::cta.b32 [%0], %1;\n" ::"r"(dst_s), "n"(NCOLS) : "memory");
}
__device__ __forceinline__ void tmem_relinquish() { asm volatile("tcgen05.relinquish_alloc_permit.cta_group::1.sync.aligned;\n" ::: "memory"); }
template <int NCOLS>
__device__ __forceinline__ void tmem_dealloc(uint32_t taddr)
{
  asm volatile("tcgen05.dealloc.cta_group::1.sync.aligned.b32 %0, %1;\n" ::"r"(taddr), "n"(NCOLS) : "memory");
}
__device__ __forceinline__ void tmem_fence_before_sync() { asm volatile("tcgen05.fence::before_thread_sync;\n" ::: "memory"); }
__device__ __forceinline__ void tmem_fence_after_sync() { asm volatile("tcgen05.fence::after_thread_sync;\n" ::: "memory"); }
__device__ __forceinline__ void tmem_st4(uint32_t taddr, const float2 (&v)[4])
{
  asm volatile("tcgen05.st.sync.aligned.32x32b.x8.b32 [%0], {%1, %2, %3, %4, %5, %6, %7, %8};\n"
               ::"r"(taddr), "f"(v[0].x), "f"(v[0].y), "f"(v[1].x), "f"(v[1].y), "f"(v[2].x), "f"(v[2].y), "f"(v[3].x), "f"(v[3].y));
}
__device__ __forceinline__ void tmem_wait_st() { asm volatile("tcgen05.wait::st.sync.aligned;\n" ::: "memory"); }
__device__ __forceinline__ void tmem_ld4(uint32_t taddr, float2 (&v)[4])
{
  asm volatile("tcgen05.ld.sync.aligned.32x32b.x8.b32 {%0, %1, %2, %3, %4, %5, %6, %7}, [%8];\n"
               : "=f"(v[0].x), "=f"(v[0].y), "=f"(v[1].x), "=f"(v[1].y), "=f"(v[2].x), "=f"(v[2].y), "=f"(v[3].x), "=f"(v[3].y)
               : "r"(taddr));
}
__device__ __forceinline__ void tmem_wait_ld4(float2 (&v)[4])
{
  asm volatile("tcgen05.wait::ld.sync.aligned;\n"
               : "+f"(v[0].x), "+f"(v[0].y), "+f"(v[1].x), "+f"(v[1].y), "+f"(v[2].x), "+f"(v[2].y), "+f"(v[3].x), "+f"(v[3].y));
}

constexpr int OFDM_FMT_MT = 2;
template <int LOG2M, int T, bool C16, int FMT, int SPLIT>
__global__ void __launch_bounds__(T, (LOG2M == 14 ? 1 : 1024 / T)) k_ofdm(const OfdmArgs a)
{
  constexpr bool MT = (FMT & OFDM_FMT_MT) != 0;
  static_assert(!MT || C16, "several constellation tables only in chain mode");
  extern __shared__ __align__(16) uint8_t smem_raw[];
  float2 *x = reinterpret_cast<float2 *>(smem_raw);
  constexpr int M = 1 << LOG2M;
  uint8_t *stage = reinterpret_cast<uint8_t *>(x + padx(M));
  float *lut_re = reinterpret_cast<float *>(stage + 2 * a.stage_cap);
  const int lut_rep_shift = a.lut_rep_shift, lut_rep = 1 << lut_rep_shift;
  const int lut_e = a.lut_n < 16 ? 16 : a.lut_n;
  float *lut_im = a.lut_single ? lut_re : lut_re + lut_e * lut_rep;
  float2 *spool = reinterpret_cast<float2 *>(lut_re + (a.lut_single ? lut_e : 2 * lut_e) * lut_rep);
  uint64_t *mbar = reinterpret_cast<uint64_t *>(spool + 8);
  const uint32_t mbar_s = (uint32_t)__cvta_generic_to_shared(mbar), dbar_s = mbar_s + 8;
  const int2 *descbuf = reinterpret_cast<const int2 *>(mbar + 2);
  const uint32_t desc_s = mbar_s + 16;
  if (C16) {
    if constexpr (MT) {
      for (int i = threadIdx.x; i < a.lut_n; i += T) x[i] = __ldg(a.lut + i);
    }
    else if (threadIdx.x < a.lut_n) x[threadIdx.x] = __ldg(a.lut + threadIdx.x);
    if (threadIdx.x < 8) spool[threadIdx.x] = __ldg(a.pool + threadIdx.x);
    if (threadIdx.x < 4) reinterpret_cast<uint32_t *>(stage)[threadIdx.x] = 0u;
    if (threadIdx.x == 0) {
      asm volatile("mbarrier.init.shared::cta.b64 [%0], 1;\n" ::"r"(mbar_s) : "memory");
      asm volatile("mbarrier.init.shared::cta.b64 [%0], 1;\n" ::"r"(dbar_s) : "memory");
      asm volatile("fence.mbarrier_init.release.cluster;\n" ::: "memory");
    }
    __syncthreads();
    for (int i = threadIdx.x; i < a.lut_n * lut_rep; i += T) {
      const float2 v = x[i >> lut_rep_shift];
      lut_re[i] = v.x;
      if (!a.lut_single) lut_im[i] = v.y;
    }
    __syncthreads();
  }
  static_assert(SPLIT == 1 || LOG2M == 14, "only 32K symbols are transformed as two halves");
  uint32_t park_col = 0;
  if constexpr (SPLIT == 2) {
    uint32_t *tm_slot = reinterpret_cast<uint32_t *>(x);
    if (threadIdx.x < 32) {
      tmem_alloc<OFDM_PARK_COLS>((uint32_t)__cvta_generic_to_shared(tm_slot));
      tmem_relinquish();
    }
    tmem_fence_before_sync();
    __syncthreads();
    tmem_fence_after_sync();
    const uint32_t warp = threadIdx.x >> 5;
    park_col = *tm_slot + ((32u * (warp & 3u)) << 16) + 64u * (warp >> 2);
  }
  constexpr int R0 = FillGeom<LOG2M, T>::R0;
  constexpr int NLAST = M / 16;
  const int N = a.fft_n;
  const int units = a.frames * a.num_symbols;
  const int cp_from = N - a.gi;
  const uint32_t stage_s = (uint32_t)__cvta_generic_to_shared(stage);
  FillSmem fs;
  fs.stage_s = stage_s;
  fs.esh = 2u + (uint32_t)lut_rep_shift;
  fs.lut_lane_s = (uint32_t)__cvta_generic_to_shared(lut_re) + ((threadIdx.x & (uint32_t)(lut_rep - 1)) << 2);
  fs.im_ofs = a.lut_single ? 0u : 4u * (uint32_t)(lut_e * lut_rep);
  fs.spool_m8_s = (uint32_t)__cvta_generic_to_shared(spool) - 8u;
  constexpr bool REGTW = LOG2M == 14;
  static_assert(!REGTW || T == 512, "the 16K schedule is written for 512 threads");
  float2 tw_p1 = make_float2(1.f, 0.f), tw_p2 = tw_p1, tw_last = tw_p1, tw_rec = tw_p1;
  if (REGTW) {
    tw_p1 = __ldg(a.tw + (threadIdx.x & 15) * (M / 256));
    tw_p2 = __ldg(a.tw + (threadIdx.x & 255) * (M / 4096));
    tw_last = __ldg(a.tw + threadIdx.x);
    if (SPLIT == 2) tw_rec = __fmul2_rn(__ldg(a.tw_split + threadIdx.x), make_float2(a.norm, a.norm));
  }
  static_assert(REGTW || M / 16 <= T, "one butterfly per thread and pass: the twiddle bases are loaded once");
  constexpr int NP1 = R0, NP2 = R0 * 16 < NLAST ? R0 * 16 : 1;
  if (!REGTW) {
    tw_p1 = __ldg(a.tw + (threadIdx.x & (NP1 - 1)) * (M / (NP1 * 16)));
    tw_p2 = __ldg(a.tw + (threadIdx.x & (NP2 - 1)) * (M / (NP2 * 16)));
    tw_last = (int)threadIdx.x < NLAST ? __ldg(a.tw + threadIdx.x) : make_float2(1.f, 0.f);
  }

  uint32_t mphase = 0, dphase = 0;
  auto run_range = [&](int u) {
    const int ul = u % a.num_symbols;
    return make_int2(__ldg(a.run_ptr + ul), __ldg(a.run_cnt + ul));
  };
  auto desc_issue = [&](int2 rr) {
    if (rr.y <= 0) return;
    const uint32_t bytes = (uint32_t)((rr.y + 1) >> 1) * 16u;
    asm volatile("mbarrier.arrive.expect_tx.shared::cta.b64 _, [%0], %1;\n" ::"r"(dbar_s), "r"(bytes) : "memory");
    asm volatile("cp.async.bulk.shared::cluster.global.mbarrier::complete_tx::bytes [%0], [%1], %2, [%3];\n"
                 ::"r"(desc_s), "l"(a.run_desc + rr.x), "r"(bytes), "r"(dbar_s) : "memory");
  };
  auto stage_issue = [&](int u, int2 rr) {
    if (rr.y <= 0) return;
    {
      uint32_t done;
      do {
        asm volatile("{\n.reg .pred p;\nmbarrier.try_wait.parity.shared::cta.b64 p, [%1], %2;\nselp.u32 %0, 1, 0, p;\n}\n"
                     : "=r"(done) : "r"(dbar_s), "r"(dphase) : "memory");
      } while (!done);
      dphase ^= 1u;
    }
    const int uf = u / a.num_symbols, ul = u - uf * a.num_symbols;
    const uint8_t *src = reinterpret_cast<const uint8_t *>(a.cells16 + (long long)uf * a.cells_stride);
    asm volatile("fence.proxy.async.shared::cta;\n" ::: "memory");
    if (threadIdx.x == 0)
      asm volatile("mbarrier.arrive.expect_tx.shared::cta.b64 _, [%0], %1;\n" ::"r"(mbar_s), "r"(__ldg(a.stage_bytes + ul)) : "memory");
#pragma unroll 2
    for (int i = threadIdx.x; i < rr.y; i += T) {
      const int2 d = descbuf[i];
      BND(i < a.desc_cap);
      BND(((unsigned)d.y >> 16) + ((unsigned)d.y & 0xFFFFu) <= (unsigned)a.stage_cap / 8u && d.x >= 0);
      BND(a.cells_len == 0 || (long long)uf * a.cells_stride * 2 + 16ll * (d.x + (d.y & 0xFFFF)) <= a.cells_len * 2 + 64);
      asm volatile("cp.async.bulk.shared::cluster.global.mbarrier::complete_tx::bytes [%0], [%1], %2, [%3];\n"
                   ::"r"(stage_s + 16u * ((uint32_t)d.y >> 16)), "l"(src + 16ll * d.x), "r"(16u * ((uint32_t)d.y & 0xFFFFu)), "r"(mbar_s) : "memory");
    }
  };
  auto stage_wait = [&]() {
    uint32_t done;
    do {
      asm volatile("{\n.reg .pred p;\nmbarrier.try_wait.parity.shared::cta.b64 p, [%1], %2;\nselp.u32 %0, 1, 0, p;\n}\n"
                   : "=r"(done) : "r"(mbar_s), "r"(mphase) : "memory");
    } while (!done);
    mphase ^= 1u;
  };

  int2 cp0 = make_int2(0, 0), cp1 = cp0;
  if (C16 && (int)blockIdx.x < units) {
    cp0 = run_range(blockIdx.x);
    if (threadIdx.x == 0) desc_issue(cp0);
  }
  for (int unit = blockIdx.x; unit < units; unit += gridDim.x) {
    const int f = unit / a.num_symbols, l = unit - f * a.num_symbols;
    if (C16 && unit + (int)gridDim.x < units) cp1 = run_range(unit + gridDim.x);
    const int variant = (a.frame_idx0 + (f % a.frames_per_channel)) % a.l1post_variants;
    const float2 *cells = a.cells + (long long)f * a.cells_stride;
    const float2 *pool = a.pool + (long long)variant * a.pool_stride;
    typedef typename SinkT<FMT & 1>::type sample_t;
    sample_t *out = reinterpret_cast<sample_t *>(a.out) + (long long)f * a.out_stride;
    sample_t *sym = out + 2048 + (long long)l * (N + a.gi);
    BND(a.out_len == 0 || (long long)f * a.out_stride + 2048 + (long long)(l + 1) * (N + a.gi) <= a.out_len);

    if (l == 0)
      for (int i = threadIdx.x; i < 2048; i += T) {
        float2 p = __ldg(a.p1 + i);
        p.x *= a.sink_gain; p.y *= a.sink_gain;
        store_sample(out, i, p);
      }

    bool pool_sym = false;
    if (C16) pool_sym = __ldg(a.sym_flags + l) != 0;
    int c[FillGeom<LOG2M, T>::GPB][FillGeom<LOG2M, T>::R0];
    fill_load_codes<LOG2M, T>(a.code_pos + (long long)l * SPLIT * M, threadIdx.x, c);
    if (C16) {
      if (unit == (int)blockIdx.x) stage_issue(unit, cp0);
      if (cp0.y > 0) stage_wait();
    }

    for (int phase = 0; phase < SPLIT; phase++) {
      const int32_t *code = a.code_pos + ((long long)l * SPLIT + phase) * M;
      const float *sinc = a.sinc_pos ? a.sinc_pos + (long long)phase * M : nullptr;
      if (phase) fill_load_codes<LOG2M, T>(code, threadIdx.x, c);
      __syncthreads();
      if (C16 && phase == 0 && threadIdx.x == 0 && unit + (int)gridDim.x < units) desc_issue(cp1);
      if (sinc) {
        if (pool_sym) ofdm_fill<LOG2M, T, C16, true, true, MT>(x, code, sinc, c, cells, pool, fs, a.stage_cap, a.lut_n);
        else ofdm_fill<LOG2M, T, C16, false, true, MT>(x, code, sinc, c, cells, pool, fs, a.stage_cap, a.lut_n);
      }
      else {
        if (pool_sym) ofdm_fill<LOG2M, T, C16, true, false, MT>(x, code, sinc, c, cells, pool, fs, a.stage_cap, a.lut_n);
        else ofdm_fill<LOG2M, T, C16, false, false, MT>(x, code, sinc, c, cells, pool, fs, a.stage_cap, a.lut_n);
      }
      __syncthreads();
      if (C16 && phase == SPLIT - 1) {
        if (unit + (int)gridDim.x < units) stage_issue(unit + gridDim.x, cp1);
        cp0 = cp1;
      }
      if constexpr (REGTW) {
        fft_pass16x2<M, 16, T>(x, tw_p1); __syncthreads();
        fft_pass16x2<M, 256, T>(x, tw_p2); __syncthreads();
      }
      else {
        if (R0 * 16 < NLAST * 16 && R0 < NLAST) { fft_pass16<M, NP1, T>(x, tw_p1); __syncthreads(); }
        if (R0 * 16 < NLAST) { fft_pass16<M, NP2, T>(x, tw_p2); __syncthreads(); }
      }
      if constexpr (REGTW) {
        constexpr int NL = M / 4, NBT = NL / T;
        constexpr int XS = NL + NL / 16;
        sample_t *o = sym + a.gi + threadIdx.x;
        const bool odd_phase = SPLIT == 2 && phase == 1;
        if (odd_phase) tmem_wait_st();
#pragma unroll
        for (int j = 0; j < NBT; j++) {
          const int i = threadIdx.x + j * T;
          const float2 *xb = x + padx(i);
          float2 e[4];
          if (odd_phase) tmem_ld4(park_col + 8u * j, e);
          float2 v[4];
#pragma unroll
          for (int q = 0; q < 4; q++) v[q] = xb[q * XS];
          const float2 w1 = j ? cmul(tw_last, w32(j)) : tw_last;
          const float2 w2 = cmul(w1, w1), w3 = cmul(w2, w1);
          v[1] = cmul(v[1], w1); v[2] = cmul(v[2], w2); v[3] = cmul(v[3], w3);
          dft_reg<4>(v);
          if (SPLIT == 1) {
            sample_t *ocp = sym + ((long long)threadIdx.x - cp_from);
#pragma unroll
            for (int k = 0; k < 4; k++) {
              const float2 r = __fmul2_rn(v[bitrev_c(k, 4)], make_float2(a.norm, a.norm));
              store_sample(o, j * T + k * NL, r);
              if (i + k * NL >= cp_from) store_sample(ocp, j * T + k * NL, r);
            }
          }
          else if (phase == 0) {
            float2 r[4];
#pragma unroll
            for (int k = 0; k < 4; k++) r[k] = __fmul2_rn(v[bitrev_c(k, 4)], make_float2(a.norm, a.norm));
            tmem_st4(park_col + 8u * j, r);
          }
          else {
            sample_t *ocp = sym + ((long long)threadIdx.x + M - cp_from);
            const float2 wi = j ? cmul(tw_rec, w64(j)) : tw_rec;
            float2 r[4];
#pragma unroll
            for (int k = 0; k < 4; k++) r[k] = cmul(tw16(v[bitrev_c(k, 4)], 2 * k), wi);
            tmem_wait_ld4(e);
#pragma unroll
            for (int k = 0; k < 4; k++) {
              store_sample(o, j * T + k * NL, cadd(e[k], r[k]));
              const float2 hi = csub(e[k], r[k]);
              store_sample(o, j * T + k * NL + M, hi);
              if (i + k * NL + M >= cp_from) store_sample(ocp, j * T + k * NL, hi);
            }
          }
        }
      }
      else
#pragma unroll 1
      for (int i = threadIdx.x; i < NLAST; i += T) {
        const float2 *xb = x + padx(i);
        float2 v[16];
#pragma unroll
        for (int qd = 0; qd < 16; qd++) v[qd] = xb[padx(qd * NLAST)];
        apply_twiddles<16>(v, tw_last);
        dft_reg<16>(v);
        sample_t *o = sym + a.gi + i;
        sample_t *ocp = sym + ((long long)i - cp_from);
#pragma unroll
        for (int k = 0; k < 16; k++) {
          float2 r = v[bitrev_c(k, 16)];
          r = __fmul2_rn(r, make_float2(a.norm, a.norm));
          store_sample(o, k * NLAST, r);
          if (i + k * NLAST >= cp_from) store_sample(ocp, k * NLAST, r);
        }
      }
    }
  }
  if constexpr (SPLIT == 2) {
    tmem_fence_before_sync();
    __syncthreads();
    if (threadIdx.x < 32) {
      tmem_fence_after_sync();
      tmem_dealloc<OFDM_PARK_COLS>(park_col);
    }
  }
}

static inline size_t lut_table_bytes(const OfdmArgs &a) { return (size_t)(a.lut_n < 16 ? 16 : a.lut_n) * 4 * (a.lut_single ? 1 : 2); }

template <int LOG2M, int T, bool C16, int FMT, int SPLIT>
static void launch_ofdm_t(const OfdmArgs &a, cudaStream_t s)
{
  constexpr int M = 1 << LOG2M;
  const size_t smem = (size_t)padx(M) * sizeof(float2) +
                      (C16 ? (size_t)a.stage_cap * 2 + ((size_t)lut_table_bytes(a) << a.lut_rep_shift) + 64 + 16 + (size_t)a.desc_cap * 8 : 0);
  const int units = a.frames * a.num_symbols;
// ... 242 lines not shown
```

gr-dvbt2ll_b200/csrc/t2_kernels.cuh:

```cuda
#ifndef T2_KERNELS_CUH
#define T2_KERNELS_CUH

#include <cuda_runtime.h>
#include <stdint.h>

namespace t2k {

struct BbArgs {
  const uint8_t *ts;
  long long ts_pitch;
  int hist_valid;
  int n_channels, frames;
  int count0;
  int fec_block0;
  int kbch, nbch, bch_r, payload_bytes, mode, inband, fecblocks;
  int chunk_bytes, lead_zero_bytes;
  const uint8_t *scramble;
  const uint8_t *crc8_tab;
  uint32_t crc8_pos_mask[47][8];
  const uint32_t *bch_tab;
  const uint32_t *bch_cols;
  const uint8_t *inband_bytes;
  uint8_t *out;
  int out_pitch;
  int out_group, out_group_stride, out_group_off;
  int *sync_errors;
  long long ts_len;
  long long out_len;
};
void launch_bb_bch(const BbArgs &a, cudaStream_t s);

struct LdpcArgs {
  const uint8_t *in;  int in_pitch;
  uint8_t *out;       int out_pitch;
  int frames;
  int nbch, nldpc, q, groups;
  const uint16_t *row_ptr;
  const uint32_t *entries;
  int lane_per_row;
  long long in_len, out_len;
};
void launch_ldpc(const LdpcArgs &a, cudaStream_t s);

struct MapArgs {
  const uint8_t *in;  int in_pitch;
  float2 *out;
  int frames;
  int nldpc, mod, cell_size, cyclic_delay;
  const uint16_t *bit_src;
  const uint2 *qpsk_lut;
  int qpsk_lin_cells;
  int qpsk_par_q, qpsk_nbch;
  const float2 *lut;
  int ncol;
  uint8_t col_of_bit[16];
  uint8_t twist_of_col[16];
  int base_of_bit[16], twist_of_bit[16];
  uint16_t *out16;
  long long out16_frame_stride;
  const uint16_t *ci_inv;
  const uint16_t *ci_inv4;
  int ci_inv4_stride;
  const int32_t *fec_shift;
  int fecblocks;
  int im_from_re;
  uint32_t im_mask_i, im_mask_q, im_flip;
  long long in_len, out_len;
};
void launch_map(const MapArgs &a, cudaStream_t s);

void launch_pack_bits(const uint8_t *in, int nbits, uint8_t *out, int out_pitch, int frames, cudaStream_t s);
void launch_unpack_bits(const uint8_t *in, int in_pitch, int nbits, uint8_t *out, int frames, cudaStream_t s);
void launch_unpack_ldpc(const uint8_t *in, int in_pitch, int nbch, int nldpc, int q, uint8_t *out, int frames,
                        cudaStream_t s);
void launch_pack_ldpc(const uint8_t *in, int nbch, int nldpc, int q, uint8_t *out, int out_pitch, int frames,
                      cudaStream_t s);

struct GatherArgs {
  const float2 *in;  long long in_stride;
  float2 *out;       long long out_stride;
  const int32_t *code; int n;
  const float2 *pool;
  int l1post_base, l1post_cells, l1post_variants;
  int frames; int frame_idx0;
};
void launch_gather(const GatherArgs &a, cudaStream_t s);

struct OfdmArgs {
  const float2 *cells; long long cells_stride;
  const uint16_t *cells16;
  const int2 *run_desc;
  const int32_t *run_ptr;
  const int32_t *run_cnt;
  int desc_cap;
  const int32_t *stage_bytes;
  const int32_t *sym_flags;
  int stage_cap;
  const float2 *lut; int lut_n;
  int lut_single;
  int lut_rep_shift;
  void *out;           long long out_stride;
  int out_fmt;
  float sink_gain;
  const int32_t *code_pos;
  const float2 *pool;
  long long pool_stride;
  int l1post_base, l1post_cells, l1post_variants;
  const float2 *p1;
  const float *sinc_pos;
  const float2 *tw;
  const float2 *tw_split;
  int fft_n, log2_m, split;
  int c_ps, left_nulls, gi, num_symbols;
  float norm;
  int frames; int frame_idx0;
  int frames_per_channel;
  long long cells_len, out_len, pool_len;
  int lut_tables;
};
constexpr int OFDM_CODE_TAB_SHIFT = 21;
constexpr unsigned OFDM_CODE_TAB_MAX = 1023;
constexpr unsigned OFDM_CODE_SMALL_POOL = 0x1E0000u;
int launch_ofdm(const OfdmArgs &a, cudaStream_t s);
int ofdm_position_of_bin(int m, int log2_m);
int ofdm_table_index(int p, int log2_m);

struct PaprArgs {
  const float2 *in;
  void *out;
  int out_fmt;
  float gain;
  int inplace;
  long long spf;
  int fft_n, gi, num_symbols, frames;
  int iterations;
  float vclip, tone_max;
  float tone_scale;
  int tones;
  const int32_t *sym_set;
  const int32_t *bins;
  const float2 *kernel;
  const float2 *tone_tw;
  int16_t *stats;
  int sets;
  long long in_len, out_len;
};
enum { PAPR_STOP_CLIP = 1, PAPR_STOP_TONE = 2, PAPR_STOP_LIMIT = 3 };
void launch_papr_tr(const PaprArgs &a, cudaStream_t s);

long long kernel_launch_count();

}
#endif
```

gr-dvbt2ll_b200/python/dvbt2ll_b200/__init__.py:

```python
import ctypes as C
import os

import numpy as np

from .configs import *
from . import configs

_HERE = os.path.dirname(os.path.abspath(__file__))
LIB_PATH = os.environ.get("DVBT2LL_LIB") or os.path.normpath(os.path.join(_HERE, "..", "..", "libdvbt2ll_cuda.so"))

_lib = None

EXPORTED_SYMBOLS = [
    "dvbt2ll_last_error", "dvbt2ll_version", "dvbt2ll_kernel_launches", "dvbt2ll_device_available",
    "dvbt2ll_output_multiple", "dvbt2ll_forecast", "dvbt2ll_work", "dvbt2ll_work_device", "dvbt2ll_warnings",
    "dvbt2ll_destroy", "dvbt2ll_plan_get", "dvbt2ll_bbheaderbch_create", "dvbt2ll_ldpc_create",
    "dvbt2ll_interleavermod_create", "dvbt2ll_framemapperfint_create", "dvbt2ll_pilotgenp1insert_create",
    "dvbt2ll_chain_create", "dvbt2ll_chain_ts_bytes_per_frame", "dvbt2ll_chain_ts_bytes", "dvbt2ll_chain_samples_per_frame",
    "dvbt2ll_chain_fecframes_per_frame", "dvbt2ll_chain_run_device", "dvbt2ll_chain_run_host",
    "dvbt2ll_chain_tap", "dvbt2ll_chain_stage_ms", "dvbt2ll_chain_enable_timing", "dvbt2ll_chain_set_sink",
    "dvbt2ll_set_overfull_policy", "dvbt2ll_set_host_register", "dvbt2ll_link", "dvbt2ll_link_hits", "dvbt2ll_link_lazy_host", "dvbt2ll_link_late_writes", "dvbt2ll_set_auto_link",
    "dvbt2ll_gather_last_error", "dvbt2ll_gather_create", "dvbt2ll_gather_export", "dvbt2ll_gather_connect",
    "dvbt2ll_gather_acquire", "dvbt2ll_gather_push", "dvbt2ll_gather_wait", "dvbt2ll_gather_release",
    "dvbt2ll_gather_side_stream", "dvbt2ll_gather_destroy",
    "dvbt2ll_copy_to_host", "dvbt2ll_copy_to_device", "dvbt2ll_device_alloc", "dvbt2ll_device_free",
    "dvbt2ll_device_count", "dvbt2ll_set_device", "dvbt2ll_device_synchronize",
    "dvbt2ll_stream_create", "dvbt2ll_stream_destroy", "dvbt2ll_stream_synchronize",
    "dvbt2ll_chain_create_multiplp", "dvbt2ll_chain_num_plp", "dvbt2ll_chain_plp_ts_bytes",
    "dvbt2ll_chain_history_bytes", "dvbt2ll_ts_sync", "dvbt2ll_ts_fill", "dvbt2ll_chain_create_plps",
    "dvbt2ll_chain_set_papr_tr",
]
GATHER_BLOB_BYTES = 256


class ChainParams(C.Structure):
    _fields_ = [(n, C.c_int) for n in (
        "framesize", "rate", "constellation", "rotation", "fecblocks", "tiblocks", "carriermode", "fftsize",
        "guardinterval", "l1constellation", "pilotpattern", "t2frames", "numdatasyms", "paprmode", "version",
        "preamble", "inputmode", "reservedbiasbits", "l1scrambled", "inband", "misogroup", "equalization",
        "bandwidth", "vlength", "tsrate")]


class PlpParams(C.Structure):
    _fields_ = [(n, C.c_int) for n in ("fecblocks", "framesize", "rate", "constellation", "rotation")]


PLP_KEYS = ("framesize", "rate", "constellation", "rotation")


def plp_params(cfg):
    return [dict({k: int(cfg[k]) for k in PLP_KEYS}, **{k: int(v) for k, v in p.items()}) for p in cfg["plps"]]


def lib():
    global _lib
    if _lib is None:
        if not os.path.exists(LIB_PATH):
            raise RuntimeError("libdvbt2ll_cuda.so not built: run `make -C gr-dvbt2ll_b200/csrc` "
                               "(or __graft_entry__.build()); there is no CPU fallback")
        L = C.CDLL(LIB_PATH)
        vp, ci, cll = C.c_void_p, C.c_int, C.c_longlong
        L.dvbt2ll_last_error.restype = C.c_char_p
        L.dvbt2ll_version.restype = C.c_char_p
        L.dvbt2ll_kernel_launches.restype = cll
        L.dvbt2ll_output_multiple.argtypes = [vp]
        L.dvbt2ll_forecast.argtypes = [vp, ci]
        L.dvbt2ll_work.argtypes = [vp, vp, ci, vp, ci, C.POINTER(ci)]
        L.dvbt2ll_work_device.argtypes = [vp, vp, ci, vp, ci, C.POINTER(ci), vp]
        L.dvbt2ll_warnings.argtypes = [vp]
        L.dvbt2ll_destroy.argtypes = [vp]
        L.dvbt2ll_plan_get.restype = cll
        L.dvbt2ll_plan_get.argtypes = [vp, C.c_char_p, vp, cll]
        for name, n in (("dvbt2ll_bbheaderbch_create", 6), ("dvbt2ll_ldpc_create", 2),
                        ("dvbt2ll_interleavermod_create", 4), ("dvbt2ll_framemapperfint_create", 20),
                        ("dvbt2ll_pilotgenp1insert_create", 12)):
            f = getattr(L, name)
            f.restype = vp
            f.argtypes = [ci] * n
        L.dvbt2ll_chain_create.restype = vp
        L.dvbt2ll_chain_create.argtypes = [C.POINTER(ChainParams), ci, ci]
        L.dvbt2ll_chain_ts_bytes_per_frame.restype = cll
        L.dvbt2ll_chain_ts_bytes_per_frame.argtypes = [vp]
        L.dvbt2ll_chain_ts_bytes.restype = cll
        L.dvbt2ll_chain_ts_bytes.argtypes = [vp, cll, ci]
        L.dvbt2ll_chain_samples_per_frame.restype = cll
        L.dvbt2ll_chain_samples_per_frame.argtypes = [vp]
        L.dvbt2ll_chain_fecframes_per_frame.argtypes = [vp]
        L.dvbt2ll_chain_run_device.argtypes = [vp, vp, cll, ci, ci, cll, vp, vp]
        L.dvbt2ll_chain_run_host.argtypes = [vp, vp, cll, ci, ci, cll, vp]
        L.dvbt2ll_chain_tap.restype = cll
        L.dvbt2ll_chain_tap.argtypes = [vp, C.c_char_p, vp, cll]
        L.dvbt2ll_chain_stage_ms.argtypes = [vp, C.POINTER(C.c_float)]
        L.dvbt2ll_chain_enable_timing.argtypes = [vp, ci]
        L.dvbt2ll_chain_set_sink.argtypes = [vp, ci, C.c_float]
        L.dvbt2ll_chain_set_papr_tr.argtypes = [vp, ci, C.c_float, C.c_float]
        L.dvbt2ll_set_overfull_policy.argtypes = [ci]
        L.dvbt2ll_set_overfull_policy.restype = None
        L.dvbt2ll_set_host_register.argtypes = [vp, ci]
        L.dvbt2ll_set_host_register.restype = None
        L.dvbt2ll_link.argtypes = [vp, vp]
        L.dvbt2ll_link_hits.argtypes = [vp]
        L.dvbt2ll_link_hits.restype = cll
        L.dvbt2ll_link_lazy_host.argtypes = [vp, ci]
        L.dvbt2ll_set_auto_link.argtypes = [ci]
        L.dvbt2ll_set_auto_link.restype = None
        L.dvbt2ll_link_late_writes.argtypes = [vp]
        L.dvbt2ll_link_late_writes.restype = cll
        sz = C.c_size_t
        L.dvbt2ll_gather_last_error.restype = C.c_char_p
        L.dvbt2ll_gather_create.restype = vp
        L.dvbt2ll_gather_create.argtypes = [ci, ci, ci, ci, sz, sz, ci]
        L.dvbt2ll_gather_export.argtypes = [vp, vp, sz]
        L.dvbt2ll_gather_connect.argtypes = [vp, vp, sz]
        L.dvbt2ll_gather_acquire.argtypes = [vp, cll, sz, vp, C.POINTER(vp)]
        L.dvbt2ll_gather_push.argtypes = [vp, cll, sz, sz, vp]
        L.dvbt2ll_gather_wait.argtypes = [vp, cll, vp, C.POINTER(vp)]
        L.dvbt2ll_gather_release.argtypes = [vp, cll, vp]
        L.dvbt2ll_gather_side_stream.restype = vp
        L.dvbt2ll_gather_side_stream.argtypes = [vp]
        L.dvbt2ll_gather_destroy.argtypes = [vp]
        L.dvbt2ll_gather_destroy.restype = None
        L.dvbt2ll_copy_to_host.argtypes = [vp, vp, sz]
        L.dvbt2ll_copy_to_device.argtypes = [vp, vp, sz]
        L.dvbt2ll_device_alloc.restype = vp
        L.dvbt2ll_device_alloc.argtypes = [sz]
        L.dvbt2ll_device_free.argtypes = [vp]
        L.dvbt2ll_device_free.restype = None
        L.dvbt2ll_set_device.argtypes = [ci]
        L.dvbt2ll_stream_create.restype = vp
        L.dvbt2ll_stream_destroy.argtypes = [vp]
        L.dvbt2ll_stream_destroy.restype = None
        L.dvbt2ll_stream_synchronize.argtypes = [vp]
        L.dvbt2ll_chain_create_multiplp.restype = vp
        L.dvbt2ll_chain_create_multiplp.argtypes = [C.POINTER(ChainParams), ci, C.POINTER(ci), ci, ci]
        L.dvbt2ll_chain_num_plp.argtypes = [vp]
        L.dvbt2ll_chain_create_plps.restype = vp
        L.dvbt2ll_chain_create_plps.argtypes = [C.POINTER(ChainParams), ci, C.POINTER(PlpParams), ci, ci]
        L.dvbt2ll_chain_plp_ts_bytes.restype = cll
        L.dvbt2ll_chain_plp_ts_bytes.argtypes = [vp, ci, cll, ci]
        L.dvbt2ll_chain_history_bytes.restype = cll
        L.dvbt2ll_chain_history_bytes.argtypes = [vp, cll]
        L.dvbt2ll_ts_sync.restype = cll
        L.dvbt2ll_ts_sync.argtypes = [vp, sz]
        L.dvbt2ll_ts_fill.restype = cll
        L.dvbt2ll_ts_fill.argtypes = [vp, sz, vp, sz, cll]
        _lib = L
    return _lib


def last_error():
    return lib().dvbt2ll_last_error().decode()


def device_available():
    return bool(lib().dvbt2ll_device_available())


def kernel_launches():
    return int(lib().dvbt2ll_kernel_launches())


def device_count():
    return int(lib().dvbt2ll_device_count())


def set_device(device):
    if lib().dvbt2ll_set_device(int(device)) < 0:
        raise RuntimeError(last_error())

# ... 369 lines not shown
```

include/dvbt2ll_cuda.h:

```cpp
#ifndef DVBT2LL_CUDA_H
#define DVBT2LL_CUDA_H

#include <stddef.h>
#include <stdint.h>

#ifdef __cplusplus
extern "C" {
#endif

#define DVBT2LL_API_EXPORT __attribute__((visibility("default")))

#define DVBT2LL_ERR_INVALID   (-1)
#define DVBT2LL_ERR_CUDA      (-2)
#define DVBT2LL_ERR_SHORT     (-3)

typedef struct dvbt2ll_handle dvbt2ll_handle;

DVBT2LL_API_EXPORT const char *dvbt2ll_last_error(void);
DVBT2LL_API_EXPORT const char *dvbt2ll_version(void);
DVBT2LL_API_EXPORT long long dvbt2ll_kernel_launches(void);
DVBT2LL_API_EXPORT int dvbt2ll_device_available(void);

DVBT2LL_API_EXPORT int dvbt2ll_output_multiple(const dvbt2ll_handle *h);
DVBT2LL_API_EXPORT int dvbt2ll_forecast(const dvbt2ll_handle *h, int noutput);
DVBT2LL_API_EXPORT int dvbt2ll_work(dvbt2ll_handle *h, const void *in, int ninput, void *out, int noutput,
                                    int *consumed);
DVBT2LL_API_EXPORT int dvbt2ll_work_device(dvbt2ll_handle *h, const void *d_in, int ninput, void *d_out,
                                           int noutput, int *consumed, void *stream);
DVBT2LL_API_EXPORT int dvbt2ll_warnings(const dvbt2ll_handle *h);
DVBT2LL_API_EXPORT void dvbt2ll_destroy(dvbt2ll_handle *h);
DVBT2LL_API_EXPORT long long dvbt2ll_plan_get(const dvbt2ll_handle *h, const char *name, void *out, long long cap);

DVBT2LL_API_EXPORT dvbt2ll_handle *dvbt2ll_bbheaderbch_create(int framesize, int rate, int mode, int inband,
                                                              int fecblocks, int tsrate);

DVBT2LL_API_EXPORT dvbt2ll_handle *dvbt2ll_ldpc_create(int framesize, int rate);

DVBT2LL_API_EXPORT dvbt2ll_handle *dvbt2ll_interleavermod_create(int framesize, int rate, int constellation,
                                                                 int rotation);

DVBT2LL_API_EXPORT dvbt2ll_handle *dvbt2ll_framemapperfint_create(
    int framesize, int rate, int constellation, int rotation, int fecblocks, int tiblocks, int carriermode,
    int fftsize, int guardinterval, int l1constellation, int pilotpattern, int t2frames, int numdatasyms,
    int paprmode, int version, int preamble, int inputmode, int reservedbiasbits, int l1scrambled, int inband);

DVBT2LL_API_EXPORT dvbt2ll_handle *dvbt2ll_pilotgenp1insert_create(
    int carriermode, int fftsize, int pilotpattern, int guardinterval, int numdatasyms, int paprmode,
    int version, int preamble, int misogroup, int equalization, int bandwidth, int vlength);

typedef struct dvbt2ll_chain_params {
  int framesize, rate, constellation, rotation, fecblocks, tiblocks, carriermode, fftsize, guardinterval,
      l1constellation, pilotpattern, t2frames, numdatasyms, paprmode, version, preamble, inputmode,
      reservedbiasbits, l1scrambled, inband, misogroup, equalization, bandwidth, vlength, tsrate;
} dvbt2ll_chain_params;

DVBT2LL_API_EXPORT dvbt2ll_handle *dvbt2ll_chain_create(const dvbt2ll_chain_params *p, int max_frames, int device);
DVBT2LL_API_EXPORT dvbt2ll_handle *dvbt2ll_chain_create_multiplp(const dvbt2ll_chain_params *p, int num_plp,
                                                                 const int *plp_fecblocks, int max_frames, int device);
typedef struct dvbt2ll_plp_params {
  int fecblocks, framesize, rate, constellation, rotation;
} dvbt2ll_plp_params;
DVBT2LL_API_EXPORT dvbt2ll_handle *dvbt2ll_chain_create_plps(const dvbt2ll_chain_params *p, int num_plp,
                                                             const dvbt2ll_plp_params *plp, int max_frames, int device);
DVBT2LL_API_EXPORT int dvbt2ll_chain_num_plp(const dvbt2ll_handle *h);
DVBT2LL_API_EXPORT long long dvbt2ll_chain_history_bytes(const dvbt2ll_handle *h, long long first_frame);
DVBT2LL_API_EXPORT long long dvbt2ll_chain_plp_ts_bytes(const dvbt2ll_handle *h, int plp, long long first_frame, int n_frames);
DVBT2LL_API_EXPORT long long dvbt2ll_chain_ts_bytes_per_frame(const dvbt2ll_handle *h);
DVBT2LL_API_EXPORT long long dvbt2ll_chain_ts_bytes(const dvbt2ll_handle *h, long long first_frame, int n_frames);
DVBT2LL_API_EXPORT long long dvbt2ll_chain_samples_per_frame(const dvbt2ll_handle *h);
DVBT2LL_API_EXPORT int dvbt2ll_chain_fecframes_per_frame(const dvbt2ll_handle *h);
DVBT2LL_API_EXPORT int dvbt2ll_chain_run_device(dvbt2ll_handle *h, const void *d_ts, long long ts_pitch,
                                                int n_channels, int n_frames, long long first_frame,
                                                void *d_out, void *stream);
DVBT2LL_API_EXPORT int dvbt2ll_chain_run_host(dvbt2ll_handle *h, const void *ts, long long ts_pitch, int n_channels,
                                              int n_frames, long long first_frame, void *out);
DVBT2LL_API_EXPORT int dvbt2ll_chain_set_sink(dvbt2ll_handle *h, int format, float gain);
DVBT2LL_API_EXPORT long long dvbt2ll_chain_tap(dvbt2ll_handle *h, const char *stage, void *out, long long cap);
DVBT2LL_API_EXPORT int dvbt2ll_chain_set_papr_tr(dvbt2ll_handle *h, int iterations, float vclip, float tone_max);
DVBT2LL_API_EXPORT int dvbt2ll_chain_stage_ms(dvbt2ll_handle *h, float *ms5);
DVBT2LL_API_EXPORT void dvbt2ll_chain_enable_timing(dvbt2ll_handle *h, int on);

DVBT2LL_API_EXPORT long long dvbt2ll_ts_sync(const unsigned char *ts, size_t n);
DVBT2LL_API_EXPORT long long dvbt2ll_ts_fill(unsigned char *dst, size_t dst_bytes, const unsigned char *src, size_t src_bytes,
                                             long long pos);

DVBT2LL_API_EXPORT int dvbt2ll_copy_to_host(void *dst, const void *d_src, size_t bytes);
DVBT2LL_API_EXPORT int dvbt2ll_copy_to_device(void *d_dst, const void *src, size_t bytes);
DVBT2LL_API_EXPORT void *dvbt2ll_device_alloc(size_t bytes);
DVBT2LL_API_EXPORT void dvbt2ll_device_free(void *p);
DVBT2LL_API_EXPORT int dvbt2ll_device_count(void);
DVBT2LL_API_EXPORT int dvbt2ll_set_device(int device);
DVBT2LL_API_EXPORT int dvbt2ll_device_synchronize(void);
DVBT2LL_API_EXPORT void *dvbt2ll_stream_create(void);
DVBT2LL_API_EXPORT void dvbt2ll_stream_destroy(void *stream);
DVBT2LL_API_EXPORT int dvbt2ll_stream_synchronize(void *stream);

DVBT2LL_API_EXPORT void dvbt2ll_set_overfull_policy(int policy);
DVBT2LL_API_EXPORT void dvbt2ll_set_host_register(dvbt2ll_handle *h, int on);
DVBT2LL_API_EXPORT int dvbt2ll_link(dvbt2ll_handle *producer, dvbt2ll_handle *consumer);
DVBT2LL_API_EXPORT void dvbt2ll_set_auto_link(int on);
DVBT2LL_API_EXPORT long long dvbt2ll_link_hits(const dvbt2ll_handle *consumer);
DVBT2LL_API_EXPORT int dvbt2ll_link_lazy_host(dvbt2ll_handle *producer, int on);
DVBT2LL_API_EXPORT long long dvbt2ll_link_late_writes(const dvbt2ll_handle *producer);

#define DVBT2LL_GATHER_BLOB_BYTES 256
typedef struct dvbt2ll_gather dvbt2ll_gather;
DVBT2LL_API_EXPORT const char *dvbt2ll_gather_last_error(void);
DVBT2LL_API_EXPORT dvbt2ll_gather *dvbt2ll_gather_create(int rank, int world, int root, int device, size_t slot_bytes,
                                                         size_t local_bytes, int n_slots);
DVBT2LL_API_EXPORT int dvbt2ll_gather_export(dvbt2ll_gather *g, void *blob, size_t cap);
DVBT2LL_API_EXPORT int dvbt2ll_gather_connect(dvbt2ll_gather *g, const void *blobs, size_t bytes);
DVBT2LL_API_EXPORT int dvbt2ll_gather_acquire(dvbt2ll_gather *g, long long step, size_t offset, void *producer_stream, void **ptr);
DVBT2LL_API_EXPORT int dvbt2ll_gather_push(dvbt2ll_gather *g, long long step, size_t offset, size_t bytes, void *producer_stream);
DVBT2LL_API_EXPORT int dvbt2ll_gather_wait(dvbt2ll_gather *g, long long step, void *consumer_stream, void **slot);
DVBT2LL_API_EXPORT int dvbt2ll_gather_release(dvbt2ll_gather *g, long long step, void *consumer_stream);
DVBT2LL_API_EXPORT void *dvbt2ll_gather_side_stream(dvbt2ll_gather *g);
DVBT2LL_API_EXPORT void dvbt2ll_gather_destroy(dvbt2ll_gather *g);

#ifdef __cplusplus
}
#endif
#endif
```

Baseline: 129,800.

## Restructure LDPC encoder with TMA bulk copies, smem tables and register shuffle prefix

Rewrites the LDPC parity kernel so that each warp prefetches the next codeword's info bits into shared memory with cp.async.bulk and an mbarrier, and writes output with bulk stores. The parity-check tables also move into shared memory. The per-row accumulators stay in registers, and the running XOR prefix is done with warp shuffles instead of a serial shared-memory scan. Lane-per-row mapping is templated (1 or 3 lanes per row), the default mode selection changes, warps per CTA drop to 2 and the grid is balanced across SMs. The aim is to overlap input loads with compute and cut shared-memory traffic, at the cost of stricter alignment requirements, a new error path and a new packed-encode API.

Result: no change. 130,300, median of 6 (+0.4%).

```diff
diff --git a/gr-dvbt2ll_b200/csrc/t2_capi.cu b/gr-dvbt2ll_b200/csrc/t2_capi.cu
--- a/gr-dvbt2ll_b200/csrc/t2_capi.cu
+++ b/gr-dvbt2ll_b200/csrc/t2_capi.cu
@@ -456,15 +456,27 @@
   }
   static int ldpc_lane_per_row_default(int nldpc, int q)
   {
-    return nldpc == 64800 ? (q >= 90 ? 1 : 0) : (q >= 18 ? 1 : 0);
+    return nldpc == 16200 && q <= 10 ? 0 : 1;
   }
   void fill_args(t2k::LdpcArgs &a, const uint8_t *in, int in_pitch, uint8_t *out, int out_pitch, int frames)
   {
     a.in = in; a.in_pitch = in_pitch; a.out = out; a.out_pitch = out_pitch; a.frames = frames;
     a.nbch = plan.fec.nbch; a.nldpc = plan.fec.nldpc; a.q = plan.fec.q; a.groups = plan.groups;
     a.row_ptr = d_rowptr.as<uint16_t>(); a.entries = d_entries.as<uint32_t>();
+    a.n_entries = (int)plan.entries.size();
     a.lane_per_row = lane_per_row;
     a.in_len = (long long)frames * in_pitch + 64; a.out_len = (long long)frames * out_pitch;
+  }
+  int encode_packed(const void *d_in, int in_pitch, void *d_out, int out_pitch, int frames, cudaStream_t s)
+  {
+    if (frames < 1) return 0;
+    t2k::LdpcArgs a;
+    fill_args(a, (const uint8_t *)d_in, in_pitch, (uint8_t *)d_out, out_pitch, frames);
+    a.in_len = a.out_len = 0;
+    if (t2k::launch_ldpc(a, s))
+      return fail(DVBT2LL_ERR_INVALID, "ldpc_encode_packed: buffers and pitches must be multiples of 16 bytes, pitches at least the codeword sizes rounded up to 16");
+    CK(cudaGetLastError());
+    return 0;
   }
   int work_device(const void *d_in, int ninput, void *d_out, int noutput, int *consumed, cudaStream_t s)
   {
@@ -478,7 +490,7 @@
     t2k::launch_pack_bits((const uint8_t *)d_in, plan.fec.nbch, d_in_packed.as<uint8_t>(), ip, frames, s);
     t2k::LdpcArgs a;
     fill_args(a, d_in_packed.as<uint8_t>(), ip, d_out_packed.as<uint8_t>(), op, frames);
-    t2k::launch_ldpc(a, s);
+    if (t2k::launch_ldpc(a, s)) return fail(DVBT2LL_ERR_INVALID, "ldpc: packed codeword buffers not 16-byte aligned");
     t2k::launch_unpack_ldpc(d_out_packed.as<uint8_t>(), op, plan.fec.nbch, plan.fec.nldpc, plan.fec.q, (uint8_t *)d_out, frames, s);
     CK(cudaGetLastError());
     if (consumed) *consumed = frames * plan.fec.nbch;
@@ -881,7 +893,10 @@
     if (!mixed()) CK(d_fec.ensure((size_t)max_frames * F() * fp + 64));
     uint8_t *fec_buf = d_fec.as<uint8_t>() + (size_t)buf_frame * F() * fp;
     uint16_t *cell_buf = d_cells.as<uint16_t>() + (size_t)buf_frame * cells16_stride();
-    if (mixed()) run_plps(d_ts, ts_pitch, n_channels, n_frames, first_frame, cell_buf, s, buf_frame, hist_valid, tev);
+    if (mixed()) {
+      const int r = run_plps(d_ts, ts_pitch, n_channels, n_frames, first_frame, cell_buf, s, buf_frame, hist_valid, tev);
+      if (r < 0) return r;
+    }
     else {
     for (int pl = 0; pl < P(); pl++) {
       const int fpl = Fp(pl);
@@ -906,7 +921,7 @@
     ma.ci_inv = d_ci_inv.as<uint16_t>(); ma.fec_shift = d_fec_shift.as<int32_t>(); ma.fecblocks = F();
     ma.ci_inv4 = d_ci_inv4.as<uint16_t>(); ma.ci_inv4_stride = ci4_stride;
     ma.out_len = (long long)frames * cells16_stride();
-    t2k::launch_ldpc(la, s);
+    if (t2k::launch_ldpc(la, s)) return fail(DVBT2LL_ERR_INVALID, "chain: FEC buffers not 16-byte aligned");
     if (timing) cudaEventRecord(tev[2], s);
     t2k::launch_map(ma, s);
     if (timing) cudaEventRecord(tev[3], s);
@@ -968,7 +983,7 @@
     tr_uploaded = true;
     return 0;
   }
-  void run_plps(const void *d_ts, long long ts_pitch, int n_channels, int n_frames, long long first_frame, uint16_t *cell_buf,
+  int run_plps(const void *d_ts, long long ts_pitch, int n_channels, int n_frames, long long first_frame, uint16_t *cell_buf,
                 cudaStream_t s, int buf_frame, int hist_valid, cudaEvent_t *tev)
   {
     const int frames = n_channels * n_frames;
@@ -989,7 +1004,7 @@
     for (int pl = 0; pl < P(); pl++) {
       t2k::LdpcArgs la;
       ldpc_of(pl).fill_args(la, bch_buf(pl), bch_pitch(pl), fec_buf(pl), fec_pitch(pl), frames * Fp(pl));
-      t2k::launch_ldpc(la, s);
+      if (t2k::launch_ldpc(la, s)) return fail(DVBT2LL_ERR_INVALID, "chain: FEC buffers not 16-byte aligned");
     }
     if (timing) cudaEventRecord(tev[2], s);
     for (int pl = 0; pl < P(); pl++) {
@@ -1004,6 +1019,7 @@
       t2k::launch_map(ma, s);
     }
     if (timing) cudaEventRecord(tev[3], s);
+    return 0;
   }
   int work_device(const void *d_in, int ninput, void *d_out, int noutput, int *consumed, cudaStream_t s)
   {
@@ -1381,6 +1397,17 @@
   std::string err;
   if (!t2::build_ldpc_plan(framesize, rate, &h->plan, &err)) { delete h; fail(DVBT2LL_ERR_INVALID, err); return 0; }
   return h;
+}
+
+int dvbt2ll_ldpc_encode_packed(dvbt2ll_handle *h, const void *d_in, int in_pitch, void *d_out, int out_pitch, int frames, void *stream)
+{
+  if (!h || h->kind != dvbt2ll_handle::LDPC) return fail(DVBT2LL_ERR_INVALID, "not an ldpc handle");
+  int r = h->enter();
+  if (r) return r;
+  cudaStream_t s = stream ? (cudaStream_t)stream : h->stream;
+  r = static_cast<LdpcHandle *>(h)->encode_packed(d_in, in_pitch, d_out, out_pitch, frames, s);
+  if (r >= 0 && !stream) CK(cudaStreamSynchronize(s));
+  return r;
 }
 
 dvbt2ll_handle *dvbt2ll_interleavermod_create(int framesize, int rate, int constellation, int rotation)
diff --git a/gr-dvbt2ll_b200/csrc/t2_kernels.cu b/gr-dvbt2ll_b200/csrc/t2_kernels.cu
--- a/gr-dvbt2ll_b200/csrc/t2_kernels.cu
+++ b/gr-dvbt2ll_b200/csrc/t2_kernels.cu
@@ -57,6 +57,35 @@
   const int k = p >> 5;
   return __funnelshift_l(w[k + 1], w[k], p & 31);
 }
+
+__device__ __forceinline__ void mbar_init(uint32_t bar)
+{
+  asm volatile("mbarrier.init.shared::cta.b64 [%0], 1;\n" ::"r"(bar) : "memory");
+}
+__device__ __forceinline__ void mbar_init_fence() { asm volatile("fence.mbarrier_init.release.cluster;\n" ::: "memory"); }
+__device__ __forceinline__ void mbar_expect_tx(uint32_t bar, uint32_t bytes)
+{
+  asm volatile("mbarrier.arrive.expect_tx.shared::cta.b64 _, [%0], %1;\n" ::"r"(bar), "r"(bytes) : "memory");
+}
+__device__ __forceinline__ void mbar_wait(uint32_t bar, uint32_t phase)
+{
+  uint32_t done;
+  do {
+    asm volatile("{\n.reg .pred p;\nmbarrier.try_wait.parity.shared::cta.b64 p, [%1], %2;\nselp.u32 %0, 1, 0, p;\n}\n"
+                 : "=r"(done) : "r"(bar), "r"(phase) : "memory");
+  } while (!done);
+}
+__device__ __forceinline__ void bulk_load(uint32_t dst, const void *src, uint32_t bytes, uint32_t bar)
+{
+  asm volatile("cp.async.bulk.shared::cluster.global.mbarrier::complete_tx::bytes [%0], [%1], %2, [%3];\n"
+               ::"r"(dst), "l"(src), "r"(bytes), "r"(bar) : "memory");
+}
+__device__ __forceinline__ void bulk_store(void *dst, uint32_t src, uint32_t bytes)
+{
+  asm volatile("cp.async.bulk.global.shared::cta.bulk_group [%0], [%1], %2;\n" ::"l"(dst), "r"(src), "r"(bytes) : "memory");
+  asm volatile("cp.async.bulk.commit_group;\n" ::: "memory");
+}
+__device__ __forceinline__ void fence_proxy_async_smem() { asm volatile("fence.proxy.async.shared::cta;\n" ::: "memory"); }
 
 constexpr int BB_MAX_WARPS = 32;
 
@@ -341,7 +370,8 @@
   count_launch();
 }
 
-constexpr int LDPC_WARPS = 3;
+constexpr int LDPC_WARPS = 2;
+constexpr int LDPC_MIN_CTAS = 7;
 
 __device__ __forceinline__ uint32_t window32_be(const uint32_t *w, int p)
 {
@@ -352,38 +382,74 @@
 __device__ __forceinline__ uint32_t be32_at(const uint32_t *w, int off)
 {
   const int k = off >> 2;
-  return __byte_perm(__ldg(w + k), __ldg(w + k + 1), 0x0123u + 0x1111u * (unsigned)(off & 3));
-}
-
-__global__ void __launch_bounds__(LDPC_WARPS * 32, 8) k_ldpc(const LdpcArgs a, int warp_words, int cw_words)
-{
+  return __byte_perm(w[k], w[k + 1], 0x0123u + 0x1111u * (unsigned)(off & 3));
+}
+
+template <int WPL>
+__device__ __forceinline__ void put_be_bytes(uint8_t *img, int B, int nb, const uint32_t (&w)[WPL])
+{
+  const int o = (4 - (B & 3)) & 3;
+  const int n = (nb - o) >> 2;
+#pragma unroll
+  for (int i = 0; i < 3; i++)
+    if (i < o) img[B + i] = (uint8_t)(w[0] >> (24 - 8 * i));
+  uint32_t *dw = reinterpret_cast<uint32_t *>(img + B + o);
+#pragma unroll
+  for (int k = 0; k < WPL; k++)
+    if (k < n) dw[k] = bswap32(__funnelshift_l(k + 1 < WPL ? w[k + 1] : 0u, w[k], 8 * o));
+#pragma unroll
+  for (int i = 0; i < 3; i++) {
+    const int b = o + 4 * n + i;
+    if (b < nb) img[B + b] = (uint8_t)(((b >> 2) == WPL - 1 ? w[WPL - 1] : w[WPL - 2]) >> (24 - 8 * (b & 3)));
+  }
+}
+
+template <int L>
+__global__ void __launch_bounds__(LDPC_WARPS * 32, LDPC_MIN_CTAS) k_ldpc(const LdpcArgs a, int slot_bytes, int warp_bytes)
+{
+  constexpr int WPL = 12 / L, RP = 32 / L;
+  constexpr int NP = (90 + RP - 1) / RP;
   extern __shared__ __align__(16) uint8_t smem_raw[];
-  uint32_t *s_all = reinterpret_cast<uint32_t *>(smem_raw);
   const int warp = threadIdx.x >> 5, lane = threadIdx.x & 31;
-  uint32_t *rows = s_all + warp * warp_words;
-  uint32_t *ext = rows + cw_words;
-  const int q = a.q, G = a.groups;
-  const int info_bytes = a.nbch / 8;
-
-  for (int job = blockIdx.x * LDPC_WARPS + warp; job < a.frames; job += gridDim.x * LDPC_WARPS) {
-    const uint8_t *in = a.in + (long long)job * a.in_pitch;
+  const int q = a.q, G = a.groups, ne = a.n_entries;
+  const int info_bytes = a.nbch / 8, cw_bytes = a.nldpc / 8;
+  const uint32_t in_bytes = (uint32_t)(info_bytes + 15) & ~15u;
+  uint32_t *s_ent = reinterpret_cast<uint32_t *>(smem_raw);
+  uint16_t *s_rp = reinterpret_cast<uint16_t *>(s_ent + ne);
+  const int tab_bytes = (ne * 4 + (q + 1) * 2 + 15) & ~15;
+  uint64_t *s_bar = reinterpret_cast<uint64_t *>(smem_raw + tab_bytes);
+  const int head = info_bytes & ~15;
+  uint8_t *inb = smem_raw + tab_bytes + LDPC_WARPS * 16 + warp * warp_bytes;
+  uint8_t *tail = inb + in_bytes;
+  uint32_t *ext = reinterpret_cast<uint32_t *>(tail + slot_bytes - head);
+  BND(q <= 90 && 45 * G == info_bytes && cw_bytes - info_bytes == 45 * q && cw_bytes <= slot_bytes && head > 0);
+  BND(warp_bytes >= (int)in_bytes + slot_bytes - head + G * 13 * 4);
+
+  for (int i = threadIdx.x; i < ne; i += blockDim.x) s_ent[i] = __ldg(a.entries + i);
+  for (int i = threadIdx.x; i <= q; i += blockDim.x) s_rp[i] = __ldg(a.row_ptr + i);
+  const uint32_t bar = (uint32_t)__cvta_generic_to_shared(s_bar + warp);
+  const uint32_t inb_s = (uint32_t)__cvta_generic_to_shared(inb), tail_s = inb_s + in_bytes;
+  if (lane == 0) {
+    mbar_init(bar);
+    mbar_init_fence();
+  }
+  __syncthreads();
+
+  const int stride = gridDim.x * LDPC_WARPS;
+  auto issue = [&](int job) {
+    BND(a.in_len == 0 || (long long)job * a.in_pitch + in_bytes <= a.in_len);
+    mbar_expect_tx(bar, in_bytes);
+    bulk_load(inb_s, a.in + (long long)job * a.in_pitch, in_bytes, bar);
+  };
+  const int job0 = blockIdx.x * LDPC_WARPS + warp;
+  if (lane == 0 && job0 < a.frames) issue(job0);
+  const int r = lane / L, s = lane - r * L;
+  int k = 0;
+  for (int job = job0; job < a.frames; job += stride, k++) {
+    const uint32_t *imgw = reinterpret_cast<const uint32_t *>(inb);
     uint8_t *out = a.out + (long long)job * a.out_pitch;
-    const uint32_t *cw = reinterpret_cast<const uint32_t *>(in);
-    BND(a.in_len == 0 || (long long)job * a.in_pitch + 45 * G + 8 <= a.in_len);
-    BND(a.out_len == 0 || (long long)job * a.out_pitch + a.nldpc / 8 <= a.out_len);
-    BND(45 * G == info_bytes && warp_words >= G * 13 + q * 12);
-    {
-      uint32_t *ow = reinterpret_cast<uint32_t *>(out);
-      const int nw = info_bytes >> 2;
-      for (int i = lane; i < nw; i += 256) {
-        uint32_t v[8];
-#pragma unroll
-        for (int u = 0; u < 8; u++) v[u] = __ldg(cw + min(i + 32 * u, nw - 1));
-#pragma unroll
-        for (int u = 0; u < 8; u++) if (i + 32 * u < nw) ow[i + 32 * u] = v[u];
-      }
-      for (int b = (nw << 2) + lane; b < info_bytes; b += 32) out[b] = __ldg(in + b);
-    }
+    BND(a.out_len == 0 || (long long)job * a.out_pitch + slot_bytes <= a.out_len);
+    mbar_wait(bar, (uint32_t)k & 1u);
     for (int idx0 = lane; idx0 < G * 13; idx0 += 128) {
       uint32_t v[4], h[4];
       int wsel[4];
@@ -392,131 +458,153 @@
         const int idx = min(idx0 + 32 * u, G * 13 - 1);
         const int g = idx / 13, w = idx - g * 13;
         wsel[u] = w;
-        v[u] = be32_at(cw, 45 * g + (w == 12 ? 3 : 4 * w));
-        h[u] = be32_at(cw, 45 * g);
+        v[u] = be32_at(imgw, 45 * g + (w == 12 ? 3 : 4 * w));
+        h[u] = be32_at(imgw, 45 * g);
       }
 #pragma unroll
       for (int u = 0; u < 4; u++)
         if (idx0 + 32 * u < G * 13) ext[idx0 + 32 * u] = wsel[u] == 11 ? (v[u] & 0xFF000000u) | (h[u] >> 8) : v[u];
     }
+    if (lane == 0) asm volatile("cp.async.bulk.wait_group.read 0;\n" ::: "memory");
     __syncwarp();
-    if (a.lane_per_row) {
-      for (int t = lane; t < q; t += 32) {
-        uint32_t acc[12];
-#pragma unroll
-        for (int w = 0; w < 12; w++) acc[w] = 0u;
-        const int e1 = a.row_ptr[t + 1];
-        for (int e = a.row_ptr[t]; e < e1; e++) {
-          const uint32_t en = __ldg(a.entries + e);
+    if (head + lane < info_bytes) tail[lane] = inb[head + lane];
+    fence_proxy_async_smem();
+    __syncwarp();
+    if (lane == 0) {
+      bulk_store(out, inb_s, (uint32_t)head);
+      if (job + stride < a.frames) {
+        asm volatile("cp.async.bulk.wait_group.read 0;\n" ::: "memory");
+        issue(job + stride);
+      }
+    }
+    uint32_t acc[NP][WPL];
+#pragma unroll
+    for (int p = 0; p < NP; p++) {
+#pragma unroll
+      for (int j = 0; j < WPL; j++) acc[p][j] = 0u;
+      const int t = p * RP + r;
+      if (p * RP < q && r < RP && t < q) {
+        const int e1 = s_rp[t + 1];
+        auto first_pos = [&](uint32_t en) {
           BND((int)(en & 0xffffu) < G && (en >> 16) < 360u);
-          const uint32_t *eg = ext + (en & 0xffffu) * 13;
-          int p = (en >> 16) ? 360 - (int)(en >> 16) : 0;
-#pragma unroll
-          for (int w = 0; w < 12; w++) {
-            acc[w] ^= window32(eg, p);
-            p += 32;
-            if (p >= 360) p -= 360;
+          const int pos = ((en >> 16) ? 360 - (int)(en >> 16) : 0) + 32 * WPL * s;
+          return pos >= 360 ? pos - 360 : pos;
+        };
+        int e = s_rp[t];
+        for (; e + 2 <= e1; e += 2) {
+          BND(e + 1 < ne);
+          const uint32_t en0 = s_ent[e], en1 = s_ent[e + 1];
+          const uint32_t *g0 = ext + (en0 & 0xffffu) * 13, *g1 = ext + (en1 & 0xffffu) * 13;
+          int p0 = first_pos(en0), p1 = first_pos(en1);
+#pragma unroll
+          for (int j = 0; j < WPL; j++) {
+            acc[p][j] ^= window32(g0, p0) ^ window32(g1, p1);
+            p0 += 32; if (p0 >= 360) p0 -= 360;
+            p1 += 32; if (p1 >= 360) p1 -= 360;
           }
         }
-        acc[11] &= 0xFF000000u;
-#pragma unroll
-        for (int w = 0; w < 12; w++) rows[t * 12 + w] = acc[w];
-      }
-    }
-    else
-    for (int idx = lane; idx < q * 12; idx += 32) {
-      const int t = idx / 12, w = idx - t * 12;
-      uint32_t acc = 0;
-      const int e1 = a.row_ptr[t + 1];
-      int e = a.row_ptr[t];
-      for (; e + 4 <= e1; e += 4) {
-        uint32_t en[4];
-#pragma unroll
-        for (int u = 0; u < 4; u++) en[u] = __ldg(a.entries + e + u);
-#pragma unroll
-        for (int u = 0; u < 4; u++) {
-          int p = 32 * w - (int)(en[u] >> 16);
-          if (p < 0) p += 360;
-          BND((int)(en[u] & 0xffffu) < G && (en[u] >> 16) < 360u && p >= 0 && p < 360);
-          acc ^= window32(ext + (en[u] & 0xffffu) * 13, p);
+        if (e < e1) {
+          BND(e < ne);
+          const uint32_t en = s_ent[e];
+          const uint32_t *eg = ext + (en & 0xffffu) * 13;
+          int pos = first_pos(en);
+#pragma unroll
+          for (int j = 0; j < WPL; j++) {
+            acc[p][j] ^= window32(eg, pos);
+            pos += 32; if (pos >= 360) pos -= 360;
+          }
         }
       }
-      for (; e < e1; e++) {
-        const uint32_t en = __ldg(a.entries + e);
-        int p = 32 * w - (int)(en >> 16);
-        if (p < 0) p += 360;
-        BND((int)(en & 0xffffu) < G && (en >> 16) < 360u && p >= 0 && p < 360);
-        acc ^= window32(ext + (en & 0xffffu) * 13, p);
-      }
-      if (w == 11) acc &= 0xFF000000u;
-      rows[idx] = acc;
-    }
-    __syncwarp();
-    if (lane < 12) {
-      uint32_t run = 0;
-      for (int t = 0; t < q; t++) { run ^= rows[t * 12 + lane]; rows[t * 12 + lane] = run; }
-    }
-    __syncwarp();
+      if (s == L - 1) acc[p][WPL - 1] &= 0xFF000000u;
+    }
+    uint32_t carry[WPL];
+#pragma unroll
+    for (int j = 0; j < WPL; j++) carry[j] = 0u;
+#pragma unroll
+    for (int p = 0; p < NP; p++) {
+      if (p * RP < q) {
+#pragma unroll
+        for (int j = 0; j < WPL; j++) {
+          uint32_t x = acc[p][j];
+#pragma unroll
+          for (int d = 1; d < RP; d <<= 1) {
+            const uint32_t o = __shfl_up_sync(0xffffffffu, x, d * L);
+            if (r >= d) x ^= o;
+          }
+          x ^= carry[j];
+          acc[p][j] = x;
+          carry[j] = __shfl_sync(0xffffffffu, x, (RP - 1) * L + s);
+        }
+      }
+    }
     uint32_t E = 0;
     {
-      uint32_t x = lane < 12 ? rows[(q - 1) * 12 + lane] : 0;
+      uint32_t x = 0;
+#pragma unroll
+      for (int j = 0; j < WPL; j++) {
+        const uint32_t v = __shfl_sync(0xffffffffu, carry[j], (lane / WPL) % L);
+        if (lane % WPL == j) x = v;
+      }
+      if (lane >= 12) x = 0;
       x ^= x >> 1; x ^= x >> 2; x ^= x >> 4; x ^= x >> 8; x ^= x >> 16;
-      uint32_t par = x & 1u, carry = par;
+      uint32_t par = x & 1u, c = par;
 #pragma unroll
       for (int d = 1; d < 16; d <<= 1) {
-        const uint32_t o = __shfl_up_sync(0xffffffffu, carry, d);
-        if (lane >= d) carry ^= o;
-      }
-      carry ^= par;
-      E = (x >> 1) ^ (carry ? 0xFFFFFFFFu : 0u);
+        const uint32_t o = __shfl_up_sync(0xffffffffu, c, d);
+        if (lane >= d) c ^= o;
+      }
+      c ^= par;
+      E = (x >> 1) ^ (c ? 0xFFFFFFFFu : 0u);
       if (lane == 11) E &= 0xFF000000u;
     }
-    for (int i0 = 0; i0 < q * 12; i0 += 32) {
-      const int idx = i0 + lane;
-      const uint32_t ew = __shfl_sync(0xffffffffu, E, idx % 12);
-      if (idx < q * 12) rows[idx] ^= ew;
-    }
+    uint32_t ew[WPL];
+#pragma unroll
+    for (int j = 0; j < WPL; j++) ew[j] = __shfl_sync(0xffffffffu, E, s * WPL + j);
+    const int seg0 = 4 * WPL * s, seg_bytes = min(4 * WPL, 45 - seg0);
+#pragma unroll
+    for (int p = 0; p < NP; p++) {
+      const int t = p * RP + r;
+      if (p * RP < q && r < RP && t < q) {
+        uint32_t w[WPL];
+#pragma unroll
+        for (int j = 0; j < WPL; j++) w[j] = acc[p][j] ^ ew[j];
+        BND(info_bytes + 45 * t + seg0 + seg_bytes <= cw_bytes);
+        put_be_bytes<WPL>(tail, info_bytes - head + 45 * t + seg0, seg_bytes, w);
+      }
+    }
+    if (cw_bytes + lane < slot_bytes) tail[cw_bytes - head + lane] = 0;
+    fence_proxy_async_smem();
     __syncwarp();
-    if ((info_bytes & 3) == 0) {
-      uint32_t *pw = reinterpret_cast<uint32_t *>(out + info_bytes);
-      const int nwp = (q * 360) >> 5;
-      for (int j = lane; j < nwp; j += 32) {
-        const int P = j << 5;
-        const int t = P / 360, o = P - t * 360;
-        uint32_t v = window32(rows + t * 12, o);
-        const int n1 = 360 - o;
-        if (n1 < 32) v = (v & ~(0xFFFFFFFFu >> n1)) | (rows[(t + 1) * 12] >> n1);
-        pw[j] = bswap32(v);
-      }
-      for (int b = (nwp << 2) + lane; b < q * 45; b += 32) {
-        const int t = b / 45, bb = b - t * 45;
-        out[info_bytes + b] = (uint8_t)(rows[t * 12 + (bb >> 2)] >> (24 - 8 * (bb & 3)));
-      }
-    }
-    else {
-      for (int b = lane; b < q * 45; b += 32) {
-        const int t = b / 45, bb = b - t * 45;
-        out[info_bytes + b] = (uint8_t)(rows[t * 12 + (bb >> 2)] >> (24 - 8 * (bb & 3)));
-      }
-    }
-    __syncwarp();
-  }
-}
-
-void launch_ldpc(const LdpcArgs &a, cudaStream_t s)
-{
-  const int cw_words = a.q * 12 + 4;
-  const int warp_words = (a.groups * 13 + cw_words + 3) & ~3;
-  const size_t smem = (size_t)LDPC_WARPS * warp_words * 4;
-  if (a.frames < 1) return;
-  static bool attr[MAX_DEVICES];
-  allow_smem(k_ldpc, 200 * 1024, attr);
+    if (lane == 0) bulk_store(out + head, tail_s, (uint32_t)(slot_bytes - head));
+  }
+  if (lane == 0) asm volatile("cp.async.bulk.wait_group 0;\n" ::: "memory");
+}
+
+int launch_ldpc(const LdpcArgs &a, cudaStream_t s)
+{
+  if (a.frames < 1) return 0;
+  const int in_bytes = (a.nbch / 8 + 15) & ~15, slot_bytes = (a.nldpc / 8 + 15) & ~15;
+  if ((reinterpret_cast<uintptr_t>(a.in) & 15) || (reinterpret_cast<uintptr_t>(a.out) & 15) || (a.in_pitch & 15) ||
+      (a.out_pitch & 15) || a.in_pitch < in_bytes || a.out_pitch < slot_bytes || a.q > 90)
+    return -1;
+  const int warp_bytes = in_bytes + slot_bytes - (a.nbch / 8 & ~15) + ((a.groups * 13 * 4 + 15) & ~15);
+  const int tab_bytes = (a.n_entries * 4 + (a.q + 1) * 2 + 15) & ~15;
+  const size_t smem = (size_t)tab_bytes + LDPC_WARPS * 16 + (size_t)LDPC_WARPS * warp_bytes;
+  static bool attr1[MAX_DEVICES], attr3[MAX_DEVICES];
+  allow_smem(k_ldpc<1>, 227 * 1024, attr1);
+  allow_smem(k_ldpc<3>, 227 * 1024, attr3);
   int per_sm = 1;
-  cudaOccupancyMaxActiveBlocksPerMultiprocessor(&per_sm, k_ldpc, LDPC_WARPS * 32, smem);
+  if (a.lane_per_row) cudaOccupancyMaxActiveBlocksPerMultiprocessor(&per_sm, k_ldpc<1>, LDPC_WARPS * 32, smem);
+  else cudaOccupancyMaxActiveBlocksPerMultiprocessor(&per_sm, k_ldpc<3>, LDPC_WARPS * 32, smem);
   if (per_sm < 1) per_sm = 1;
-  const int blocks = (a.frames + LDPC_WARPS - 1) / LDPC_WARPS;
-  k_ldpc<<<blocks, LDPC_WARPS * 32, smem, s>>>(a, warp_words, cw_words);
+  const int cap = per_sm * sm_count();
+  const int ctas = (a.frames + LDPC_WARPS - 1) / LDPC_WARPS;
+  const int rounds = (ctas + cap - 1) / cap;
+  const int blocks = (ctas + rounds - 1) / rounds;
+  if (a.lane_per_row) k_ldpc<1><<<blocks, LDPC_WARPS * 32, smem, s>>>(a, slot_bytes, warp_bytes);
+  else k_ldpc<3><<<blocks, LDPC_WARPS * 32, smem, s>>>(a, slot_bytes, warp_bytes);
   count_launch();
+  return 0;
 }
 
 constexpr int MAP_THREADS = 128;
@@ -1489,9 +1577,9 @@
     if (threadIdx.x < 8) spool[threadIdx.x] = __ldg(a.pool + threadIdx.x);
     if (threadIdx.x < 4) reinterpret_cast<uint32_t *>(stage)[threadIdx.x] = 0u;
     if (threadIdx.x == 0) {
-      asm volatile("mbarrier.init.shared::cta.b64 [%0], 1;\n" ::"r"(mbar_s) : "memory");
-      asm volatile("mbarrier.init.shared::cta.b64 [%0], 1;\n" ::"r"(dbar_s) : "memory");
-      asm volatile("fence.mbarrier_init.release.cluster;\n" ::: "memory");
+      mbar_init(mbar_s);
+      mbar_init(dbar_s);
+      mbar_init_fence();
     }
     __syncthreads();
     for (int i = threadIdx.x; i < a.lut_n * lut_rep; i += T) {
@@ -1552,41 +1640,28 @@
   auto desc_issue = [&](int2 rr) {
     if (rr.y <= 0) return;
     const uint32_t bytes = (uint32_t)((rr.y + 1) >> 1) * 16u;
-    asm volatile("mbarrier.arrive.expect_tx.shared::cta.b64 _, [%0], %1;\n" ::"r"(dbar_s), "r"(bytes) : "memory");
-    asm volatile("cp.async.bulk.shared::cluster.global.mbarrier::complete_tx::bytes [%0], [%1], %2, [%3];\n"
-                 ::"r"(desc_s), "l"(a.run_desc + rr.x), "r"(bytes), "r"(dbar_s) : "memory");
+    mbar_expect_tx(dbar_s, bytes);
+    bulk_load(desc_s, a.run_desc + rr.x, bytes, dbar_s);
   };
   auto stage_issue = [&](int u, int2 rr) {
     if (rr.y <= 0) return;
-    {
-      uint32_t done;
-      do {
-        asm volatile("{\n.reg .pred p;\nmbarrier.try_wait.parity.shared::cta.b64 p, [%1], %2;\nselp.u32 %0, 1, 0, p;\n}\n"
-                     : "=r"(done) : "r"(dbar_s), "r"(dphase) : "memory");
-      } while (!done);
-      dphase ^= 1u;
-    }
+    mbar_wait(dbar_s, dphase);
+    dphase ^= 1u;
     const int uf = u / a.num_symbols, ul = u - uf * a.num_symbols;
     const uint8_t *src = reinterpret_cast<const uint8_t *>(a.cells16 + (long long)uf * a.cells_stride);
-    asm volatile("fence.proxy.async.shared::cta;\n" ::: "memory");
-    if (threadIdx.x == 0)
-      asm volatile("mbarrier.arrive.expect_tx.shared::cta.b64 _, [%0], %1;\n" ::"r"(mbar_s), "r"(__ldg(a.stage_bytes + ul)) : "memory");
+    fence_proxy_async_smem();
+    if (threadIdx.x == 0) mbar_expect_tx(mbar_s, __ldg(a.stage_bytes + ul));
 #pragma unroll 2
     for (int i = threadIdx.x; i < rr.y; i += T) {
       const int2 d = descbuf[i];
       BND(i < a.desc_cap);
       BND(((unsigned)d.y >> 16) + ((unsigned)d.y & 0xFFFFu) <= (unsigned)a.stage_cap / 8u && d.x >= 0);
       BND(a.cells_len == 0 || (long long)uf * a.cells_stride * 2 + 16ll * (d.x + (d.y & 0xFFFF)) <= a.cells_len * 2 + 64);
-      asm volatile("cp.async.bulk.shared::cluster.global.mbarrier::complete_tx::bytes [%0], [%1], %2, [%3];\n"
-                   ::"r"(stage_s + 16u * ((uint32_t)d.y >> 16)), "l"(src + 16ll * d.x), "r"(16u * ((uint32_t)d.y & 0xFFFFu)), "r"(mbar_s) : "memory");
+      bulk_load(stage_s + 16u * ((uint32_t)d.y >> 16), src + 16ll * d.x, 16u * ((uint32_t)d.y & 0xFFFFu), mbar_s);
     }
   };
   auto stage_wait = [&]() {
-    uint32_t done;
-    do {
-      asm volatile("{\n.reg .pred p;\nmbarrier.try_wait.parity.shared::cta.b64 p, [%1], %2;\nselp.u32 %0, 1, 0, p;\n}\n"
-                   : "=r"(done) : "r"(mbar_s), "r"(mphase) : "memory");
-    } while (!done);
+    mbar_wait(mbar_s, mphase);
     mphase ^= 1u;
   };
 
diff --git a/gr-dvbt2ll_b200/csrc/t2_kernels.cuh b/gr-dvbt2ll_b200/csrc/t2_kernels.cuh
--- a/gr-dvbt2ll_b200/csrc/t2_kernels.cuh
+++ b/gr-dvbt2ll_b200/csrc/t2_kernels.cuh
@@ -37,10 +37,11 @@
   int nbch, nldpc, q, groups;
   const uint16_t *row_ptr;
   const uint32_t *entries;
+  int n_entries;
   int lane_per_row;
   long long in_len, out_len;
 };
-void launch_ldpc(const LdpcArgs &a, cudaStream_t s);
+int launch_ldpc(const LdpcArgs &a, cudaStream_t s);
 
 struct MapArgs {
   const uint8_t *in;  int in_pitch;
diff --git a/gr-dvbt2ll_b200/python/dvbt2ll_b200/__init__.py b/gr-dvbt2ll_b200/python/dvbt2ll_b200/__init__.py
--- a/gr-dvbt2ll_b200/python/dvbt2ll_b200/__init__.py
+++ b/gr-dvbt2ll_b200/python/dvbt2ll_b200/__init__.py
@@ -14,7 +14,7 @@
 EXPORTED_SYMBOLS = [
     "dvbt2ll_last_error", "dvbt2ll_version", "dvbt2ll_kernel_launches", "dvbt2ll_device_available",
     "dvbt2ll_output_multiple", "dvbt2ll_forecast", "dvbt2ll_work", "dvbt2ll_work_device", "dvbt2ll_warnings",
-    "dvbt2ll_destroy", "dvbt2ll_plan_get", "dvbt2ll_bbheaderbch_create", "dvbt2ll_ldpc_create",
+    "dvbt2ll_destroy", "dvbt2ll_plan_get", "dvbt2ll_bbheaderbch_create", "dvbt2ll_ldpc_create", "dvbt2ll_ldpc_encode_packed",
     "dvbt2ll_interleavermod_create", "dvbt2ll_framemapperfint_create", "dvbt2ll_pilotgenp1insert_create",
     "dvbt2ll_chain_create", "dvbt2ll_chain_ts_bytes_per_frame", "dvbt2ll_chain_ts_bytes", "dvbt2ll_chain_samples_per_frame",
     "dvbt2ll_chain_fecframes_per_frame", "dvbt2ll_chain_run_device", "dvbt2ll_chain_run_host",
diff --git a/include/dvbt2ll_cuda.h b/include/dvbt2ll_cuda.h
--- a/include/dvbt2ll_cuda.h
+++ b/include/dvbt2ll_cuda.h
@@ -35,6 +35,8 @@
                                                               int fecblocks, int tsrate);
 
 DVBT2LL_API_EXPORT dvbt2ll_handle *dvbt2ll_ldpc_create(int framesize, int rate);
+DVBT2LL_API_EXPORT int dvbt2ll_ldpc_encode_packed(dvbt2ll_handle *h, const void *d_in, int in_pitch, void *d_out,
+                                                  int out_pitch, int frames, void *stream);
 
 DVBT2LL_API_EXPORT dvbt2ll_handle *dvbt2ll_interleavermod_create(int framesize, int rate, int constellation,
                                                                  int rotation);
```
